# choderalab/pymbar

Hardware: NVIDIA H100
Metric: MBAR self-consistent iteration throughput at K=256, N=1e7 samples per GPU (u_kn entries/s; iter/s and HBM GB/s alongside) (higher is better)
Workload: dtype f64

## Files before the change

pymbar_b200/csrc/api.cu:

```cuda
#include <dlfcn.h>
#include <nccl.h>

#include <algorithm>
#include <cmath>
#include <cstring>

#include "internal.cuh"

using namespace mbar;

namespace mbar {

struct NcclApi {
    void* handle = nullptr;
    ncclResult_t (*GetUniqueId)(ncclUniqueId*) = nullptr;
    ncclResult_t (*CommInitRank)(ncclComm_t*, int, ncclUniqueId, int) = nullptr;
    ncclResult_t (*CommDestroy)(ncclComm_t) = nullptr;
    ncclResult_t (*AllReduce)(const void*, void*, size_t, ncclDataType_t, ncclRedOp_t, ncclComm_t,
                              cudaStream_t) = nullptr;
    const char* (*GetErrorString)(ncclResult_t) = nullptr;
};
static NcclApi g_nccl;

static int nccl_load() {
// ... 94 lines not shown
    const bool wantL = want.L || want.G || want.Gall;
    bool fused = false, wroteW = false;
    for (int attempt = 0; attempt < 3; ++attempt) {
        fused = false;
        wroteW = false;
        const bool logAll = (attempt == 2);
        if (attempt == 0 && c->kernelChoice != MBAR_B200_KERNEL_GENERIC)
            MBAR_TRY(launch_pass_fused(c, f, wantL, needUnsampled, &fused, want.G && !want.Gall, &wroteW));
        if (attempt == 0 && !fused) continue;
        if (!fused) MBAR_TRY(launch_pass_generic(c, f, wantL, logAll));
        MBAR_TRY(comm_allreduce(c, c->d_out, K + 2, 0));
        if (((needUnsampled && !fused) || logAll) && c->comm && c->nranks > 1) {
            double* mx = c->d_scratch;
            double* sc = c->d_scratch + K;
            MBAR_CUDA(cudaMemcpyAsync(mx, c->d_out + lay.logS(), K * sizeof(double),
                                      cudaMemcpyDeviceToDevice, c->stream));
            MBAR_TRY(comm_allreduce(c, mx, K, 2));
            logs_to_scaled<<<(K + 255) / 256, 256, 0, c->stream>>>(c->d_out + lay.logS(), mx, sc, K);
            MBAR_TRY(comm_allreduce(c, sc, K, 0));
            scaled_to_logs<<<(K + 255) / 256, 256, 0, c->stream>>>(c->d_out + lay.logS(), mx, sc, K);
            c->launches += 2;
        }
        MBAR_CUDA(cudaMemcpyAsync(c->h_out, c->d_out, (size_t)lay.size(false) * sizeof(double),
                                  cudaMemcpyDeviceToHost, c->stream));
        MBAR_CUDA(cudaStreamSynchronize(c->stream));
        c->d2hBytes += (int64_t)lay.size(false) * 8;
        float ms = 0.f;
        if (event_ms(c->evA, c->evB, &ms)) c->lastPassMs = ms;
        if (fused && c->h_out[lay.flag()] != 0.0) continue;
        if (fused && needUnsampled) {
            bool ok = true;
            for (int k = 0; k < K; ++k)
                if (!(c->h_Nk[k] > 0)) {
                    const double S = c->h_out[lay.S() + k];
                    if (!(S > 1e-250 && S < 1e12)) ok = false;
                    c->h_out[lay.logS() + k] = std::log(S);
                    c->h_out[lay.S() + k] = 0.0;
                }
            if (!ok) continue;
        }
        if (logAll) {
            for (int k : c->active) c->h_out[lay.S() + k] = std::exp(c->h_out[lay.logS() + k]);
            break;
        }
        bool underflow = false;
        for (int k : c->active) {
            const double S = c->h_out[lay.S() + k];
            if (!(S > 1e-280)) underflow = true;
            c->h_out[lay.logS() + k] = std::log(S);
        }
        if (!underflow) break;
        if (attempt == 0) ++attempt;
    }
    if (needUnsampled)
        for (int k = 0; k < K; ++k)
            if (!(c->h_Nk[k] > 0) && c->h_ufar[k] != 0.0 && c->h_uclamp[k] == 0.0) c->h_out[lay.logS() + k] = -INFINITY;
    if (want.G || want.Gall) {
        NvtxRange nvtxH("mbar_b200::hessian");
        MBAR_TRY(launch_hessian(c, f, want.Gall, fused && wroteW));
        MBAR_TRY(comm_allreduce(c, c->d_out + lay.G(), K * K, 0));
        MBAR_CUDA(cudaMemcpyAsync(c->h_out + lay.G(), c->d_out + lay.G(), (size_t)K * K * sizeof(double),
                                  cudaMemcpyDeviceToHost, c->stream));
        MBAR_CUDA(cudaStreamSynchronize(c->stream));
        c->d2hBytes += (int64_t)K * K * 8;
    }
    return MBAR_B200_OK;
}

double global_sumx(mbar_b200_ctx* c, int* rc) {
    *rc = MBAR_B200_OK;
    const double mine = c->d_wgt ? c->sumXw : c->sumX;
    if (!c->comm || c->nranks == 1) return mine;
    double* d = c->d_scratch;
    cudaMemcpyAsync(d, &mine, sizeof(double), cudaMemcpyHostToDevice, c->stream);
    *rc = comm_allreduce(c, d, 1, 0);
    double v = 0.0;
    cudaMemcpyAsync(&v, d, sizeof(double), cudaMemcpyDeviceToHost, c->stream);
    cudaStreamSynchronize(c->stream);
    return v;
}

}

extern "C" {

int mbar_b200_pass(mbar_b200_ctx* c, const double* f, double* S, double* sumL, double* G) {
    PassWant w;
    w.G = (G != nullptr);
    MBAR_TRY(run_pass(c, f, w));
    const int K = c->K;
    const PassLayout lay{K};
    if (S) std::memcpy(S, c->h_out + lay.S(), K * sizeof(double));
    if (sumL) {
        int rc;
        const double sx = global_sumx(c, &rc);
        MBAR_TRY(rc);
        *sumL = c->h_out[lay.sumL()] - sx;
    }
    if (G) {
        const double* Gh = c->h_out + lay.G();
        for (int i = 0; i < K; ++i)
            for (int j = 0; j < K; ++j) {
                const double d = c->h_Nk[i] * c->h_Nk[j];
                G[(size_t)i * K + j] = d > 0 ? Gh[(size_t)i * K + j] / d : 0.0;
            }
    }
    return MBAR_B200_OK;
}

int mbar_b200_pass_multi(mbar_b200_ctx* c, int32_t M, const double* f, double* S, double* sumL) {
    MBAR_REQUIRE(c && f, MBAR_B200_ERR_INVALID, "NULL argument");
    MBAR_REQUIRE(M >= 1 && M <= 2, MBAR_B200_ERR_INVALID, "M=%d: 1 or 2 candidates", M);
    MBAR_REQUIRE(c->ready, MBAR_B200_ERR_NOT_READY, "u_kn has not been uploaded");
    MBAR_REQUIRE(c->nranks == 1 || c->comm, MBAR_B200_ERR_NOT_READY, "sharded problem without a communicator");
    MBAR_CUDA(cudaSetDevice(c->device));
    const int K = c->K;
    const PassLayout lay{K};
    NvtxRange nvtx_("mbar_b200::pass_multi");
    for (int m = 0; m < M; ++m) MBAR_TRY(check_range(c, f + (size_t)m * K));
    int rc0;
    const double sx = global_sumx(c, &rc0);
    MBAR_TRY(rc0);
    bool fast = c->kernelChoice != MBAR_B200_KERNEL_GENERIC;
    FusedParams p[2];
    bool batched = false;
    static const bool noM2 = std::getenv("MBAR_B200_NO_M2") != nullptr;
    if (fast && M == 2 && !noM2) {
        bool ok0 = false, ok1 = false;
        MBAR_TRY(fused_prepare(c, f, false, false, &p[0], &ok0, c->dc(ROW_C), c->hf(ROW_C), false, 2));
        if (ok0)
            MBAR_TRY(fused_prepare(c, f + K, false, false, &p[1], &ok1, c->dc(ROW_C2), c->hf(ROW_C2), false, 2));
        if (ok0 && ok1) {
            p[0].c2 = p[1].c;
            p[0].mid2 = p[1].mid;
            p[0].out = c->d_outM;
            p[0].out2 = c->d_outM + lay.size(false);
            batched = true;
        }
    }
    for (int m = 0; m < M && fast && !batched; ++m) {
        bool ok = false;
        const int row = m == 0 ? ROW_C : ROW_C2;
        MBAR_TRY(fused_prepare(c, f + (size_t)m * K, false, false, &p[m], &ok, c->dc(row), c->hf(row)));
        p[m].out = c->d_outM + (size_t)m * lay.size(false);
        fast = ok;
    }
    if (fast) {
        if (batched) {
            MBAR_TRY(fused_enqueue(c, p[0]));
            MBAR_TRY(comm_allreduce(c, p[0].out, K + 2, 0));
            MBAR_TRY(comm_allreduce(c, p[0].out2, K + 2, 0));
        } else {
            for (int m = 0; m < M; ++m) {
                MBAR_TRY(fused_enqueue(c, p[m]));
                MBAR_TRY(comm_allreduce(c, p[m].out, K + 2, 0));
            }
        }
        MBAR_CUDA(cudaMemcpyAsync(c->h_out, c->d_outM, (size_t)M * lay.size(false) * sizeof(double),
                                  cudaMemcpyDeviceToHost, c->stream));
        MBAR_CUDA(cudaStreamSynchronize(c->stream));
        c->d2hBytes += (int64_t)M * lay.size(false) * 8;
        for (int m = 0; m < M && fast; ++m) {
            const double* o = c->h_out + (size_t)m * lay.size(false);
            if (o[lay.flag()] != 0.0) fast = false;
            for (int k : c->active)
                if (!(o[k] > 1e-280)) fast = false;
        }
        if (fast) {
            for (int m = 0; m < M; ++m) {
                const double* o = c->h_out + (size_t)m * lay.size(false);
                if (S)
                    for (int k = 0; k < K; ++k) S[(size_t)m * K + k] = c->h_Nk[k] > 0 ? o[k] : 0.0;
                if (sumL) sumL[m] = o[lay.sumL()] - sx;
            }
            return MBAR_B200_OK;
        }
    }
    for (int m = 0; m < M; ++m) {
        MBAR_TRY(run_pass(c, f + (size_t)m * K, PassWant{}));
        if (S) std::memcpy(S + (size_t)m * K, c->h_out + lay.S(), K * sizeof(double));
        if (sumL) sumL[m] = c->h_out[lay.sumL()] - sx;
    }
    return MBAR_B200_OK;
}

int mbar_b200_last_kernels(const mbar_b200_ctx* c, char* pass_kernel, char* hessian_kernel, int32_t len) {
    MBAR_REQUIRE(c && len > 0, MBAR_B200_ERR_INVALID, "bad argument");
    if (pass_kernel) snprintf(pass_kernel, (size_t)len, "%s", c->lastKernel);
    if (hessian_kernel) snprintf(hessian_kernel, (size_t)len, "%s", c->lastHessKernel);
    return MBAR_B200_OK;
}

int mbar_b200_last_hessian_ms(mbar_b200_ctx* c, double* weights_ms, double* hessian_ms) {
    MBAR_REQUIRE(c, MBAR_B200_ERR_INVALID, "ctx is NULL");
    MBAR_CUDA(cudaSetDevice(c->device));
    MBAR_CUDA(cudaStreamSynchronize(c->stream));
    float a = 0.f, b = 0.f;
    if (cudaEventElapsedTime(&a, c->evH0, c->evH1) != cudaSuccess) { cudaGetLastError(); a = 0.f; }
    if (cudaEventElapsedTime(&b, c->evH1, c->evH2) != cudaSuccess) { cudaGetLastError(); b = 0.f; }
    if (weights_ms) *weights_ms = a;
    if (hessian_ms) *hessian_ms = b;
    return MBAR_B200_OK;
}

int mbar_b200_self_consistent_update(mbar_b200_ctx* c, const double* f, double* f_out) {
    MBAR_REQUIRE(f_out, MBAR_B200_ERR_INVALID, "f_out is NULL");
    PassWant w;
    w.unsampled = true;
    MBAR_TRY(run_pass(c, f, w));
    const PassLayout lay{c->K};
    for (int k = 0; k < c->K; ++k) {
        f_out[k] = f[k] - c->h_out[lay.logS() + k];
    }
    return MBAR_B200_OK;
}

int mbar_b200_gradient(mbar_b200_ctx* c, const double* f, double* g_out) {
    MBAR_REQUIRE(g_out, MBAR_B200_ERR_INVALID, "g_out is NULL");
    MBAR_TRY(run_pass(c, f, PassWant{}));
    for (int k = 0; k < c->K; ++k) g_out[k] = c->h_Nk[k] * (c->h_out[k] - 1.0);
    return MBAR_B200_OK;
}

int mbar_b200_objective_and_gradient(mbar_b200_ctx* c, const double* f, double* obj, double* g_out) {
    MBAR_REQUIRE(obj, MBAR_B200_ERR_INVALID, "obj_out is NULL");
    MBAR_TRY(run_pass(c, f, PassWant{}));
    const PassLayout lay{c->K};
    int rc;
    const double sx = global_sumx(c, &rc);
    MBAR_TRY(rc);
    double nf = 0.0;
    for (int k = 0; k < c->K; ++k) nf += c->h_Nk[k] * f[k];
    *obj = (c->h_out[lay.sumL()] - sx) - nf;
    if (g_out)
        for (int k = 0; k < c->K; ++k) g_out[k] = c->h_Nk[k] * (c->h_out[k] - 1.0);
    return MBAR_B200_OK;
}

int mbar_b200_hessian(mbar_b200_ctx* c, const double* f, double* H) {
    MBAR_REQUIRE(H, MBAR_B200_ERR_INVALID, "H_out is NULL");
    PassWant w;
    w.G = true;
    MBAR_TRY(run_pass(c, f, w));
    const int K = c->K;
    const PassLayout lay{K};
    const double* Gh = c->h_out + lay.G();
    for (int i = 0; i < K; ++i)
        for (int j = 0; j < K; ++j) {
            double v = -Gh[(size_t)i * K + j];
            if (i == j) v += c->h_Nk[i] * c->h_out[lay.S() + i];
            H[(size_t)i * K + j] = (c->h_Nk[i] > 0 && c->h_Nk[j] > 0) ? v : 0.0;
        }
    return MBAR_B200_OK;
}

int mbar_b200_weight_moments(mbar_b200_ctx* c, const double* f, double* S, double* G) {
    MBAR_REQUIRE(G, MBAR_B200_ERR_INVALID, "G_out is NULL");
    PassWant w;
    w.unsampled = true;
    w.Gall = true;
    MBAR_TRY(run_pass(c, f, w));
    const int K = c->K;
    const PassLayout lay{K};
    const double* Gh = c->h_out + lay.G();
    for (int i = 0; i < K; ++i) {
        const double si = c->h_Nk[i] > 0 ? c->h_Nk[i] : 1.0;
        if (S) S[i] = c->h_Nk[i] > 0 ? c->h_out[lay.S() + i] : std::exp(c->h_out[lay.logS() + i]);
        for (int j = 0; j < K; ++j) {
            const double sj = c->h_Nk[j] > 0 ? c->h_Nk[j] : 1.0;
            G[(size_t)i * K + j] = Gh[(size_t)i * K + j] / (si * sj);
        }
    }
    return MBAR_B200_OK;
}

int mbar_b200_log_W_nk(mbar_b200_ctx* c, const double* f, double* logW, int64_t ld, int expo) {
    MBAR_REQUIRE(logW, MBAR_B200_ERR_INVALID, "logW_host is NULL");
    MBAR_REQUIRE(c && ld >= c->K, MBAR_B200_ERR_INVALID, "ld_out < K");
    PassWant w;
    w.L = true;
    MBAR_TRY(run_pass(c, f, w));
    return launch_logw(c, f, logW, ld, expo, 0, c->N);
}

int mbar_b200_log_W_nk_rows(mbar_b200_ctx* c, const double* f, int64_t n0, int64_t n, double* logW, int64_t ld,
                            int expo) {
    MBAR_REQUIRE(logW, MBAR_B200_ERR_INVALID, "logW_host is NULL");
    MBAR_REQUIRE(c && ld >= c->K, MBAR_B200_ERR_INVALID, "ld_out < K");
    MBAR_REQUIRE(n0 >= 0 && n >= 1 && n0 + n <= c->N && n0 % TILE_N == 0, MBAR_B200_ERR_INVALID,
                 "rows [%lld, +%lld): n0 must be a multiple of 32 inside [0, N_local)", (long long)n0, (long long)n);
    PassWant w;
    w.L = true;
    MBAR_TRY(run_pass(c, f, w));
    return launch_logw(c, f, logW, ld, expo, n0, n);
}

int mbar_b200_log_denominator(mbar_b200_ctx* c, const double* f, double* L_host) {
    MBAR_REQUIRE(L_host, MBAR_B200_ERR_INVALID, "L_host is NULL");
    PassWant w;
    w.L = true;
    MBAR_TRY(run_pass(c, f, w));
    std::vector<double> x((size_t)c->N);
    MBAR_CUDA(cudaMemcpyAsync(L_host, c->d_L, (size_t)c->N * sizeof(double), cudaMemcpyDeviceToHost, c->stream));
    MBAR_CUDA(cudaMemcpyAsync(x.data(), c->d_xshift, (size_t)c->N * sizeof(double), cudaMemcpyDeviceToHost, c->stream));
    MBAR_CUDA(cudaStreamSynchronize(c->stream));
    c->d2hBytes += 2 * c->N * 8;
// ... 99 lines not shown
```

pymbar_b200/csrc/ctx.cu:

```cuda
#include <cmath>
#include <cstring>
#include <algorithm>
#include <cstdlib>
#include <condition_variable>
#include <functional>
#include <mutex>
#include <thread>

#include <sys/syscall.h>
#include <unistd.h>

#include "internal.cuh"

namespace mbar {

static thread_local char g_err[512] = "";

namespace {
struct HostPool {
    std::vector<std::thread> workers;
    std::mutex m;
    std::condition_variable cvStart, cvDone;
    const std::function<void(int)>* fn = nullptr;
    int nTasks = 0, next = 0, running = 0;
    uint64_t generation = 0;
    bool stop = false;
    int width = 1;

    HostPool() {
        int hw = (int)std::thread::hardware_concurrency();
        width = std::max(1, std::min(16, hw));
        if (const char* v = std::getenv("MBAR_B200_HOST_THREADS")) width = std::max(1, std::min(64, std::atoi(v)));
        for (int t = 1; t < width; ++t) workers.emplace_back([this] { loop(); });
    }
    ~HostPool() {
        {
            std::lock_guard<std::mutex> g(m);
            stop = true;
        }
        cvStart.notify_all();
        for (auto& w : workers) w.join();
    }
    void drain(std::unique_lock<std::mutex>& lk) {
        while (next < nTasks) {
            const int i = next++;
            ++running;
            lk.unlock();
            (*fn)(i);
            lk.lock();
            --running;
        }
    }
    void loop() {
        std::unique_lock<std::mutex> lk(m);
        uint64_t seen = 0;
        for (;;) {
            cvStart.wait(lk, [&] { return stop || generation != seen; });
            if (stop) return;
            seen = generation;
            drain(lk);
            if (running == 0 && next >= nTasks) cvDone.notify_all();
        }
    }
    void run(int n, const std::function<void(int)>& f) {
        std::unique_lock<std::mutex> lk(m);
        fn = &f;
        nTasks = n;
        next = 0;
        ++generation;
        cvStart.notify_all();
        drain(lk);
        cvDone.wait(lk, [&] { return running == 0 && next >= nTasks; });
        fn = nullptr;
    }
};
HostPool& pool() {
    static HostPool p;
    return p;
}
std::mutex g_poolUse;
}

void host_parallel(int nTasks, const std::function<void(int)>& fn) {
    if (nTasks <= 1) {
        for (int i = 0; i < nTasks; ++i) fn(i);
        return;
    }
    std::lock_guard<std::mutex> g(g_poolUse);
    pool().run(nTasks, fn);
}
int host_parallel_width() { return pool().width; }

int gpu_numa_node(int device) {
    static int cache[16] = {-2, -2, -2, -2, -2, -2, -2, -2, -2, -2, -2, -2, -2, -2, -2, -2};
    int& c = cache[device & 15];
    if (c != -2) return c;
    c = -1;
    char bus[32] = "";
    if (cudaDeviceGetPCIBusId(bus, sizeof(bus), device) != cudaSuccess) {
        cudaGetLastError();
        return c;
    }
    for (char* q = bus; *q; ++q)
        if (*q >= 'A' && *q <= 'F') *q = (char)(*q - 'A' + 'a');
    char path[128];
    snprintf(path, sizeof(path), "/sys/bus/pci/devices/%s/numa_node", bus);
    if (FILE* fh = fopen(path, "r")) {
        int node = -1;
        if (fscanf(fh, "%d", &node) == 1) c = node;
        fclose(fh);
    }
    return c;
}
NumaPrefer::NumaPrefer(int device) {
#if defined(SYS_set_mempolicy)
    const int node = gpu_numa_node(device);
    if (node < 0 || node >= 1024) return;
    unsigned long mask[16] = {0};
    mask[node / (8 * sizeof(unsigned long))] |= 1ul << (node % (8 * sizeof(unsigned long)));
    if (syscall(SYS_set_mempolicy, 1, mask, (unsigned long)(sizeof(mask) * 8)) == 0) active = true;
#else
    (void)device;
#endif
}
NumaPrefer::~NumaPrefer() {
#if defined(SYS_set_mempolicy)
    if (active) syscall(SYS_set_mempolicy, 0 , nullptr, 0ul);
#endif
}

void set_error(const char* fmt, ...) {
    va_list ap;
    va_start(ap, fmt);
    vsnprintf(g_err, sizeof(g_err), fmt, ap);
    va_end(ap);
}

struct Parked {
    void* ptr = nullptr;
    size_t bytes = 0;
};
struct DevicePool {
    Parked u, stageDev[2], stagePin[2];
};
static DevicePool g_pool[16];
static std::mutex g_poolMutex;
static bool pool_enabled() {
    static const bool off = std::getenv("MBAR_B200_NO_POOL") != nullptr;
    return !off;
}
static void* pool_take(Parked& slot, size_t bytes) {
    std::lock_guard<std::mutex> g(g_poolMutex);
    if (slot.ptr && slot.bytes >= bytes && slot.bytes <= 2 * bytes + (1u << 20)) {
        void* p = slot.ptr;
        slot = Parked{};
        return p;
    }
    return nullptr;
}
static void* pool_park(Parked& slot, void* ptr, size_t bytes) {
    std::lock_guard<std::mutex> g(g_poolMutex);
    void* old = slot.ptr;
    slot.ptr = ptr;
    slot.bytes = bytes;
    return old;
}

__device__ __forceinline__ void row_min_push(int* rowMin, double v, int lane) {
    int vi = v < 0.0 ? (int)fmax(floor(v), -1073741824.0) : 0;
    vi = __reduce_min_sync(0xffffffffu, vi);
    if (lane == 0 && vi < 0) atomicMin(rowMin, vi);
}
__device__ __forceinline__ void row_clamp_push(int* rowClamp, unsigned long long* rowFar, double d, bool valid,
                                               int lane) {
    const unsigned far = __ballot_sync(0xffffffffu, valid && d >= U_NEAR_CLAMP);
    if (far == 0u) return;
    const bool finite = __any_sync(0xffffffffu, valid && d >= U_NEAR_CLAMP && d < INFINITY);
    if (lane == 0) {
        atomicAdd(rowFar, (unsigned long long)__popc(far));
        if (finite) atomicOr(rowClamp, 1);
    }
}

enum { BAD_NAN = 1, BAD_NO_FINITE = 2, BAD_NEG_INF = 4 };
static const char* upload_error(int flags) {
    return flags & BAD_NAN ? "u_kn contains NaN"
         : flags & BAD_NO_FINITE ? "a sample has no finite energy in any sampled state"
                                 : "an unsampled state has an energy of -inf (its free energy would be -inf)";
}

__global__ void __launch_bounds__(256) retile_kernel(const double* __restrict__ src, int64_t ld,
                                                     int K, int64_t tile0, int64_t validCols,
                                                     const unsigned long long* __restrict__ rowmask,
                                                     double* __restrict__ dst,
                                                     double* __restrict__ xshift,
                                                     int* __restrict__ flags, int* __restrict__ urowmin,
                                                     unsigned long long* __restrict__ urowfar) {
    __shared__ double s_min[8][TILE_N];
    __shared__ int s_bad[8];
    const int lane = threadIdx.x & 31, warp = threadIdx.x >> 5;
    const int64_t tileLocal = blockIdx.x;
    const int64_t col = tileLocal * TILE_N + lane;
    const bool valid = col < validCols;
    const double* colp = src + col;

    double mn = INFINITY;
    unsigned bad = 0;
    for (int k = warp; k < K; k += 8) {
        double v = valid ? colp[(int64_t)k * ld] : 0.0;
        if (v != v) bad |= BAD_NAN;
        const bool act = (rowmask[k >> 6] >> (k & 63)) & 1ull;
        if (act) mn = fmin(mn, v);
        else if (v == -INFINITY) bad |= BAD_NEG_INF;
    }
    s_min[warp][lane] = mn;
    bad = __reduce_or_sync(0xffffffffu, bad);
    if (lane == 0) s_bad[warp] = (int)bad;
    __syncthreads();
    double x = s_min[0][lane];
#pragma unroll
    for (int w = 1; w < 8; ++w) x = fmin(x, s_min[w][lane]);
    int anyBad = 0;
#pragma unroll
    for (int w = 0; w < 8; ++w) anyBad |= s_bad[w];
    const bool finiteShift = isfinite(x);
    if (valid && !finiteShift && warp == 0) atomicOr(&flags[0], BAD_NO_FINITE);
    if (!valid || !finiteShift) x = 0.0;

    double* out = dst + (tile0 + tileLocal) * (int64_t)K * TILE_N + lane;
    for (int k = warp; k < K; k += 8) {
        double v = valid ? colp[(int64_t)k * ld] : 0.0;
        const double d = v - x;
        row_clamp_push(urowmin + K + k, urowfar + k, d, valid, lane);
        v = fmin(d, U_CLAMP);
        row_min_push(urowmin + k, valid ? v : 0.0, lane);
        out[(int64_t)k * TILE_N] = valid ? v : 0.0;
    }
    if (warp == 0) xshift[(tile0 + tileLocal) * TILE_N + lane] = x;
    if (anyBad && threadIdx.x == 0) atomicOr(&flags[0], anyBad);
}

int retile_chunk(mbar_b200_ctx* ctx, const double* d_rowmajor, int64_t ldCols, int64_t tile0,
                 int64_t nTilesChunk, int64_t validCols, cudaStream_t s) {
    if (nTilesChunk <= 0) return MBAR_B200_OK;
    retile_kernel<<<(unsigned)nTilesChunk, 256, 0, s>>>(d_rowmajor, ldCols, ctx->K, tile0, validCols,
                                                       ctx->d_rowmask, ctx->d_u, ctx->d_xshift,
                                                       ctx->d_flag, ctx->d_urowmin, ctx->d_urowfar);
    ctx->launches++;
    MBAR_CUDA(cudaGetLastError());
    return MBAR_B200_OK;
}

__global__ void __launch_bounds__(256) untile_kernel(const double* __restrict__ u,
                                                     const double* __restrict__ xshift, int K,
                                                     int64_t n0, int64_t n, double* __restrict__ dst,
                                                     int64_t ld) {
    const int lane = threadIdx.x & 31, warp = threadIdx.x >> 5;
    const int64_t j = (int64_t)blockIdx.x * TILE_N + lane;
    if (j >= n) return;
    const int64_t g = n0 + j;
    const int64_t tile = g / TILE_N;
    const int l = (int)(g % TILE_N);
    const double x = xshift[g];
    for (int k = warp; k < K; k += 8)
        dst[(int64_t)k * ld + j] = u[(tile * K + k) * TILE_N + l] + x;
}

int launch_untile(mbar_b200_ctx* ctx, int64_t n0, int64_t n, double* d_dst, int64_t ld) {
    const unsigned grid = (unsigned)((n + TILE_N - 1) / TILE_N);
    untile_kernel<<<grid, 256, 0, ctx->stream>>>(ctx->d_u, ctx->d_xshift, ctx->K, n0, n, d_dst, ld);
    ctx->launches++;
    MBAR_CUDA(cudaGetLastError());
    return MBAR_B200_OK;
}

__global__ void __launch_bounds__(256) sumx_kernel(const double* __restrict__ x, int64_t N,
                                                   double* __restrict__ partial) {
    __shared__ double s[8];
    double acc = 0.0;
    for (int64_t i = (int64_t)blockIdx.x * blockDim.x + threadIdx.x; i < N;
         i += (int64_t)gridDim.x * blockDim.x)
        acc += x[i];
    acc = warp_sum(acc);
    if ((threadIdx.x & 31) == 0) s[threadIdx.x >> 5] = acc;
    __syncthreads();
    if (threadIdx.x == 0) {
        double t = 0.0;
        for (int w = 0; w < 8; ++w) t += s[w];
        partial[blockIdx.x] = t;
    }
}

__global__ void __launch_bounds__(256) wprep_kernel(const double* __restrict__ w, const double* __restrict__ x,
                                                    int64_t N, double* __restrict__ sqrtw,
                                                    double* __restrict__ partial) {
    __shared__ double s[8];
    double acc = 0.0;
    for (int64_t i = (int64_t)blockIdx.x * blockDim.x + threadIdx.x; i < N;
         i += (int64_t)gridDim.x * blockDim.x) {
        const double wi = w[i];
        sqrtw[i] = sqrt(wi);
        acc += wi * x[i];
    }
    acc = warp_sum(acc);
    if ((threadIdx.x & 31) == 0) s[threadIdx.x >> 5] = acc;
    __syncthreads();
    if (threadIdx.x == 0) {
        double t = 0.0;
        for (int i = 0; i < 8; ++i) t += s[i];
        partial[blockIdx.x] = t;
    }
}

int set_weights(mbar_b200_ctx* ctx, const double* w_host) {
    if (!w_host) {
        cudaFree(ctx->d_wgt);
        cudaFree(ctx->d_sqrtw);
        ctx->d_wgt = ctx->d_sqrtw = nullptr;
// ... 138 lines not shown
}

int open_device(int device, cudaDeviceProp* propOut) {
    int ndev = 0;
    if (cudaGetDeviceCount(&ndev) != cudaSuccess || ndev == 0) {
        cudaGetLastError();
        set_error("no CUDA device visible: libmbar_b200 has no CPU fallback");
        return MBAR_B200_ERR_NO_DEVICE;
    }
    MBAR_REQUIRE(device >= 0 && device < ndev, MBAR_B200_ERR_INVALID, "device %d of %d", device, ndev);
    MBAR_CUDA(cudaSetDevice(device));
    cudaDeviceProp prop;
    MBAR_CUDA(cudaGetDeviceProperties(&prop, device));
    if (prop.major != 9 || prop.minor != 0) {
        set_error("device %d is sm_%d%d; this library is built for sm_90a (H100) only", device,
                  prop.major, prop.minor);
        return MBAR_B200_ERR_NO_DEVICE;
    }
    if (propOut) *propOut = prop;
    return MBAR_B200_OK;
}

}

using namespace mbar;

extern "C" {

int mbar_b200_abi_version(void) { return MBAR_B200_ABI_VERSION; }
const char* mbar_b200_last_error(void) { return g_err; }

int mbar_b200_device_count(int* count) {
    MBAR_REQUIRE(count, MBAR_B200_ERR_INVALID, "count is NULL");
    int n = 0;
    cudaError_t e = cudaGetDeviceCount(&n);
    if (e != cudaSuccess) {
        cudaGetLastError();
        n = 0;
    }
    *count = n;
    return MBAR_B200_OK;
}

int mbar_b200_host_alloc(void** ptr, uint64_t bytes) {
    MBAR_REQUIRE(ptr, MBAR_B200_ERR_INVALID, "ptr is NULL");
    int dev = 0;
    cudaGetDevice(&dev);
    NumaPrefer numa(dev);
    MBAR_CUDA(cudaHostAlloc(ptr, bytes, cudaHostAllocDefault));
    return MBAR_B200_OK;
}
int mbar_b200_host_free(void* ptr) {
    if (ptr) MBAR_CUDA(cudaFreeHost(ptr));
    return MBAR_B200_OK;
}

static inline uint64_t mix64(uint64_t h, uint64_t w) {
    h ^= w;
    h *= 0x9E3779B97F4A7C15ull;
    return h ^ (h >> 29);
}
static uint64_t hash_span(const unsigned char* p, size_t bytes, uint64_t seed) {
    uint64_t h0 = seed, h1 = seed ^ 0xD6E8FEB86659FD93ull, h2 = seed + 0xA0761D6478BD642Full, h3 = ~seed;
    size_t i = 0;
    for (; i + 32 <= bytes; i += 32) {
        uint64_t w[4];
        std::memcpy(w, p + i, 32);
        h0 = mix64(h0, w[0]);
        h1 = mix64(h1, w[1]);
        h2 = mix64(h2, w[2]);
        h3 = mix64(h3, w[3]);
    }
    for (; i < bytes; ++i) h0 = mix64(h0, p[i]);
    return mix64(mix64(mix64(h0, h1), h2), h3);
}

int mbar_b200_host_hash(const void* base, int64_t rows, int64_t row_bytes, int64_t stride_bytes, uint64_t* out) {
    MBAR_REQUIRE(base && out && rows >= 0 && row_bytes >= 0 && stride_bytes >= row_bytes, MBAR_B200_ERR_INVALID,
                 "bad argument");
    const unsigned char* b = static_cast<const unsigned char*>(base);
    const int64_t blk = 4ll << 20;
    const int64_t perRow = row_bytes ? (row_bytes + blk - 1) / blk : 0;
    const int64_t nBlocks = rows * perRow;
    std::vector<uint64_t> part((size_t)nBlocks);
    host_parallel((int)std::min<int64_t>(nBlocks, 1 << 30), [&](int i) {
        const int64_t r = i / perRow, c = i % perRow;
        const int64_t off = c * blk, len = std::min(blk, row_bytes - off);
        part[(size_t)i] = hash_span(b + r * stride_bytes + off, (size_t)len, 0x243F6A8885A308D3ull + (uint64_t)i);
    });
    uint64_t h = 0x13198A2E03707344ull ^ (uint64_t)rows ^ ((uint64_t)row_bytes << 20);
    for (uint64_t v : part) h = mix64(h, v);
    *out = h;
    return MBAR_B200_OK;
}

int mbar_b200_create(mbar_b200_ctx** out, int device, int32_t K, int64_t N_local, const double* N_k) {
    MBAR_REQUIRE(out && N_k, MBAR_B200_ERR_INVALID, "NULL argument");
    *out = nullptr;
    MBAR_REQUIRE(K >= 1 && K <= MBAR_B200_MAX_STATES, MBAR_B200_ERR_INVALID, "K=%d outside [1, %d]", K,
                 MBAR_B200_MAX_STATES);
    MBAR_REQUIRE(N_local >= 1, MBAR_B200_ERR_INVALID, "N_local=%lld must be >= 1", (long long)N_local);
    cudaDeviceProp prop;
    MBAR_TRY(open_device(device, &prop));
    mbar_b200_ctx* c = new mbar_b200_ctx();
    c->device = device;
    c->K = K;
    c->N = N_local;
    c->nTiles = (N_local + TILE_N - 1) / TILE_N;
    c->smCount = prop.multiProcessorCount;
    c->h_Nk.assign(N_k, N_k + K);
    c->h_logNk.resize(K);
    c->h_logNkEff.resize(K);
    std::vector<unsigned long long> mask((K + 63) / 64, 0ull);
    for (int k = 0; k < K; ++k) {
        if (!(N_k[k] >= 0.0)) {
            delete c;
            set_error("N_k[%d]=%g is negative or NaN", k, N_k[k]);
            return MBAR_B200_ERR_INVALID;
        }
        c->N_total_states += N_k[k];
        if (N_k[k] > 0) {
            c->active.push_back(k);
            mask[k >> 6] |= 1ull << (k & 63);
            c->h_logNk[k] = std::log(N_k[k]);
            c->h_logNkEff[k] = c->h_logNk[k];
        } else {
            c->h_logNk[k] = -INFINITY;
            c->h_logNkEff[k] = LOG_EPS_UNSAMPLED;
        }
    }
    if (c->active.empty()) {
        delete c;
        set_error("all N_k are zero");
        return MBAR_B200_ERR_INVALID;
    }
    c->firstActive = c->active[0];

    const size_t uBytes = (size_t)c->nTiles * K * TILE_N * sizeof(double);
    const size_t nPad = (size_t)c->nTiles * TILE_N;
    const PassLayout lay{K};
#define ALLOC(p, bytes)                                                        \
    do {                                                                       \
        cudaError_t e = cudaMalloc((void**)&(p), (bytes));                     \
        if (e != cudaSuccess) {                                                \
            set_error("cudaMalloc(%zu bytes) failed: %s", (size_t)(bytes), cudaGetErrorString(e)); \
            mbar_b200_destroy(c);                                              \
            return MBAR_B200_ERR_NOMEM;                                        \
        }                                                                      \
    } while (0)
    c->uBytes = uBytes;
    if (pool_enabled()) {
        c->d_u = static_cast<double*>(pool_take(g_pool[device & 15].u, uBytes));
        if (c->d_u) c->uBytes = 0;
    }
    if (!c->d_u) ALLOC(c->d_u, uBytes);
    ALLOC(c->d_xshift, nPad * sizeof(double));
    ALLOC(c->d_c, DC_ROWS * (size_t)K * sizeof(double));
    ALLOC(c->d_Nk, (size_t)K * sizeof(double));
    ALLOC(c->d_NkEff, (size_t)K * sizeof(double));
    ALLOC(c->d_rowmask, mask.size() * sizeof(unsigned long long));
    ALLOC(c->d_zeromask, mask.size() * sizeof(unsigned long long));
    ALLOC(c->d_onesmask, mask.size() * sizeof(unsigned long long));
    ALLOC(c->d_partial, (size_t)MAX_GRID * (3 * (size_t)K + 2) * sizeof(double));
    ALLOC(c->d_out, (size_t)lay.size(true) * sizeof(double));
    ALLOC(c->d_ticket, 4 * sizeof(unsigned int));
    ALLOC(c->d_flag, 4 * sizeof(int));
    ALLOC(c->d_urowmin, 2 * (size_t)K * sizeof(int));
    ALLOC(c->d_urowfar, (size_t)K * sizeof(unsigned long long));
    c->h_urowmin.assign(K, 0.0);
    c->h_uclamp.assign(K, 0.0);
    c->h_ufar.assign(K, 0.0);
    ALLOC(c->d_f, (size_t)K * sizeof(double));
    ALLOC(c->d_scratch, (scratch_rendezvous(K) + 1024) * sizeof(double));
    ALLOC(c->d_loop, sizeof(mbar::LoopState));
    ALLOC(c->d_av, 8 * (size_t)K * sizeof(double));
    ALLOC(c->d_outM, 2 * (size_t)lay.size(false) * sizeof(double));
    ALLOC(c->d_A, (size_t)K * K * sizeof(double));
    ALLOC(c->d_active, (size_t)K * sizeof(int));
    ALLOC(c->d_seq, sizeof(unsigned long long));
#undef ALLOC
#define CREATE_CUDA(call)                                                                   \
    do {                                                                                    \
        cudaError_t e__ = (call);                                                           \
        if (e__ != cudaSuccess) {                                                           \
            set_error("%s failed at %s:%d: %s", #call, __FILE__, __LINE__,                  \
                      cudaGetErrorString(e__));                                             \
            mbar_b200_destroy(c);                                                           \
            return MBAR_B200_ERR_CUDA;                                                      \
        }                                                                                   \
    } while (0)
    CREATE_CUDA(cudaHostAlloc((void**)&c->h_loop, sizeof(mbar::LoopState), cudaHostAllocDefault));
    CREATE_CUDA(cudaMemset(c->d_loop, 0, sizeof(mbar::LoopState)));
    CREATE_CUDA(cudaMemset(c->d_seq, 0, sizeof(unsigned long long)));
    CREATE_CUDA(cudaMemcpy(c->d_active, c->active.data(), c->active.size() * sizeof(int), cudaMemcpyHostToDevice));
    CREATE_CUDA(cudaEventCreate(&c->evH0));
    CREATE_CUDA(cudaEventCreate(&c->evH1));
    CREATE_CUDA(cudaEventCreate(&c->evH2));
    CREATE_CUDA(cudaHostAlloc((void**)&c->h_out,
                              (size_t)std::max(lay.size(true), 2 * lay.size(false)) * sizeof(double),
                              cudaHostAllocDefault));
    CREATE_CUDA(cudaHostAlloc((void**)&c->h_f, HF_ROWS * (size_t)K * sizeof(double), cudaHostAllocDefault));
    CREATE_CUDA(cudaStreamCreateWithFlags(&c->stream, cudaStreamNonBlocking));
    CREATE_CUDA(cudaStreamCreateWithFlags(&c->copyStream, cudaStreamNonBlocking));
    CREATE_CUDA(cudaEventCreate(&c->evA));
    CREATE_CUDA(cudaEventCreate(&c->evB));
    CREATE_CUDA(cudaEventCreateWithFlags(&c->evCopy[0], cudaEventDisableTiming));
    CREATE_CUDA(cudaEventCreateWithFlags(&c->evCopy[1], cudaEventDisableTiming));
    CREATE_CUDA(cudaMemcpy(c->d_Nk, N_k, (size_t)K * sizeof(double), cudaMemcpyHostToDevice));
    {
        std::vector<double> eff(K);
        for (int k = 0; k < K; ++k) eff[k] = std::exp(c->h_logNkEff[k]);
        CREATE_CUDA(cudaMemcpy(c->d_NkEff, eff.data(), (size_t)K * sizeof(double), cudaMemcpyHostToDevice));
    }
    CREATE_CUDA(cudaMemcpy(c->d_rowmask, mask.data(), mask.size() * sizeof(unsigned long long),
                         cudaMemcpyHostToDevice));
    CREATE_CUDA(cudaMemset(c->d_zeromask, 0, mask.size() * sizeof(unsigned long long)));
    CREATE_CUDA(cudaMemset(c->d_onesmask, 0xff, mask.size() * sizeof(unsigned long long)));
    CREATE_CUDA(cudaMemset(c->d_ticket, 0, 4 * sizeof(unsigned int)));
    CREATE_CUDA(cudaMemset(c->d_flag, 0, 4 * sizeof(int)));
    CREATE_CUDA(cudaMemset(c->d_urowmin, 0, 2 * (size_t)K * sizeof(int)));
    CREATE_CUDA(cudaMemset(c->d_urowfar, 0, (size_t)K * sizeof(unsigned long long)));
#undef CREATE_CUDA
    *out = c;
    return MBAR_B200_OK;
}

int mbar_b200_destroy(mbar_b200_ctx* c) {
    if (!c) return MBAR_B200_OK;
    cudaSetDevice(c->device);
    if (c->comm) mbar_b200_comm_destroy(c);
    for (void* pm : c->peerMapped) cudaIpcCloseMemHandle(pm);
    cudaFree(c->d_inbox);
    if (c->stream) cudaStreamSynchronize(c->stream);
    if (pool_enabled() && c->d_u) {
        const size_t need = (size_t)c->nTiles * c->K * TILE_N * sizeof(double);
        cudaFree(pool_park(g_pool[c->device & 15].u, c->d_u, c->uBytes ? c->uBytes : need));
        for (int i = 0; i < 2; ++i) {
            const size_t sb = (size_t)c->stageCols * c->K * sizeof(double);
            if (c->stage_dev[i]) cudaFree(pool_park(g_pool[c->device & 15].stageDev[i], c->stage_dev[i], sb));
            if (c->stage_pinned[i]) {
                void* old = pool_park(g_pool[c->device & 15].stagePin[i], c->stage_pinned[i], sb);
                if (old) cudaFreeHost(old);
            }
            c->stage_dev[i] = nullptr;
            c->stage_pinned[i] = nullptr;
        }
    } else {
        cudaFree(c->d_u);
    }
    cudaFree(c->d_xshift); cudaFree(c->d_wgt); cudaFree(c->d_sqrtw); cudaFree(c->d_c); cudaFree(c->d_Nk); cudaFree(c->d_NkEff);
    cudaFree(c->d_rowmask); cudaFree(c->d_zeromask); cudaFree(c->d_onesmask); cudaFree(c->d_partial); cudaFree(c->d_out); cudaFree(c->d_L);
    cudaFree(c->d_W); cudaFree(c->d_ticket); cudaFree(c->d_flag); cudaFree(c->d_urowmin); cudaFree(c->d_urowfar); cudaFree(c->d_f);
    cudaFree(c->d_scratch);
    cudaFree(c->d_loop); cudaFree(c->d_av); cudaFree(c->d_outM); cudaFree(c->d_A); cudaFree(c->d_active);
    cudaFree(c->d_seq); cudaFree(c->d_Wt);
    if (c->loopGraph) cudaGraphExecDestroy(c->loopGraph);
    if (c->h_loop) cudaFreeHost(c->h_loop);
    if (c->evH0) cudaEventDestroy(c->evH0);
    if (c->evH1) cudaEventDestroy(c->evH1);
    if (c->evH2) cudaEventDestroy(c->evH2);
    for (int i = 0; i < 2; ++i) {
        if (c->stage_pinned[i]) cudaFreeHost(c->stage_pinned[i]);
        cudaFree(c->stage_dev[i]);
        if (c->evCopy[i]) cudaEventDestroy(c->evCopy[i]);
    }
    if (c->h_out) cudaFreeHost(c->h_out);
    if (c->h_f) cudaFreeHost(c->h_f);
    if (c->evA) cudaEventDestroy(c->evA);
    if (c->evB) cudaEventDestroy(c->evB);
    if (c->stream) cudaStreamDestroy(c->stream);
    if (c->copyStream) cudaStreamDestroy(c->copyStream);
    cudaGetLastError();
    delete c;
    return MBAR_B200_OK;
}

int mbar_b200_trim(void) {
    int cur = 0;
    cudaGetDevice(&cur);
    for (int d = 0; d < 16; ++d) {
        DevicePool old;
        {
            std::lock_guard<std::mutex> g(g_poolMutex);
            old = g_pool[d];
            g_pool[d] = DevicePool{};
        }
        if (!old.u.ptr && !old.stageDev[0].ptr && !old.stageDev[1].ptr && !old.stagePin[0].ptr &&
            !old.stagePin[1].ptr)
            continue;
        cudaSetDevice(d);
        cudaFree(old.u.ptr);
        for (int i = 0; i < 2; ++i) {
            cudaFree(old.stageDev[i].ptr);
            if (old.stagePin[i].ptr) cudaFreeHost(old.stagePin[i].ptr);
        }
    }
    cudaSetDevice(cur);
    cudaGetLastError();
    return MBAR_B200_OK;
}

int mbar_b200_get_shape(const mbar_b200_ctx* c, int32_t* K, int64_t* N_local) {
    MBAR_REQUIRE(c, MBAR_B200_ERR_INVALID, "ctx is NULL");
    if (K) *K = c->K;
    if (N_local) *N_local = c->N;
    return MBAR_B200_OK;
}

int mbar_b200_set_pass_kernel(mbar_b200_ctx* c, int kernel) {
    MBAR_REQUIRE(c, MBAR_B200_ERR_INVALID, "ctx is NULL");
    MBAR_REQUIRE(kernel >= 0 && kernel <= 2, MBAR_B200_ERR_INVALID, "kernel=%d", kernel);
    c->kernelChoice = kernel;
    return MBAR_B200_OK;
}

int mbar_b200_get_counters(const mbar_b200_ctx* c, int64_t* launches, int64_t* passes,
                           int64_t* h2d, int64_t* d2h) {
    MBAR_REQUIRE(c, MBAR_B200_ERR_INVALID, "ctx is NULL");
    if (launches) *launches = c->launches;
    if (passes) *passes = c->passes;
    if (h2d) *h2d = c->h2dBytes;
    if (d2h) *d2h = c->d2hBytes;
    return MBAR_B200_OK;
}

int mbar_b200_last_pass_ms(mbar_b200_ctx* c, double* ms) {
    MBAR_REQUIRE(c && ms, MBAR_B200_ERR_INVALID, "NULL argument");
    cudaSetDevice(c->device);
    float t = 0.f;
    if (c->stream && cudaStreamSynchronize(c->stream) == cudaSuccess && event_ms(c->evA, c->evB, &t))
        c->lastPassMs = t;
    else
        cudaGetLastError();
    *ms = c->lastPassMs;
    return MBAR_B200_OK;
}

static int ensure_staging(mbar_b200_ctx* c, bool needPinned) {
    if (c->stageCols == 0) {
        int64_t cols = (64ll << 20) / (8ll * c->K);
        cols = (cols / TILE_N) * TILE_N;
        if (cols < TILE_N) cols = TILE_N;
        const int64_t padN = c->nTiles * TILE_N;
        if (cols > padN) cols = padN;
        c->stageCols = cols;
    }
    const size_t bytes = (size_t)c->stageCols * c->K * sizeof(double);
    for (int i = 0; i < 2; ++i) {
        if (!c->stage_dev[i] && pool_enabled())
            c->stage_dev[i] = static_cast<double*>(pool_take(g_pool[c->device & 15].stageDev[i], bytes));
        if (!c->stage_dev[i]) MBAR_CUDA(cudaMalloc((void**)&c->stage_dev[i], bytes));
        if (needPinned && !c->stage_pinned[i] && pool_enabled())
            c->stage_pinned[i] = static_cast<double*>(pool_take(g_pool[c->device & 15].stagePin[i], bytes));
        if (needPinned && !c->stage_pinned[i]) {
            NumaPrefer numa(c->device);
            MBAR_CUDA(cudaHostAlloc((void**)&c->stage_pinned[i], bytes, cudaHostAllocDefault));
        }
    }
    return MBAR_B200_OK;
}

static int reset_row_stats(mbar_b200_ctx* c) {
    MBAR_CUDA(cudaMemset(c->d_urowmin, 0, 2 * (size_t)c->K * sizeof(int)));
    MBAR_CUDA(cudaMemset(c->d_urowfar, 0, (size_t)c->K * sizeof(unsigned long long)));
    return MBAR_B200_OK;
}

static int collect_row_minima(mbar_b200_ctx* c) {
    std::vector<int> m(2 * (size_t)c->K);
    std::vector<unsigned long long> far(c->K);
    MBAR_CUDA(cudaMemcpy(m.data(), c->d_urowmin, m.size() * sizeof(int), cudaMemcpyDeviceToHost));
    MBAR_CUDA(cudaMemcpy(far.data(), c->d_urowfar, far.size() * sizeof(unsigned long long), cudaMemcpyDeviceToHost));
    MBAR_TRY(reset_row_stats(c));
    for (int k = 0; k < c->K; ++k) {
        c->h_urowmin[k] = (double)m[k];
        c->h_uclamp[k] = (double)m[c->K + k];
        c->h_ufar[k] = far[k] == (unsigned long long)c->N ? 1.0 : 0.0;
    }
    return agree_row_minima(c);
}

static int finish_upload(mbar_b200_ctx* c) {
    int flags[4];
    MBAR_CUDA(cudaStreamSynchronize(c->copyStream));
    MBAR_CUDA(cudaStreamSynchronize(c->stream));
    MBAR_CUDA(cudaMemcpy(flags, c->d_flag, sizeof(flags), cudaMemcpyDeviceToHost));
    if (flags[0]) {
        MBAR_CUDA(cudaMemset(c->d_flag, 0, 4 * sizeof(int)));
        MBAR_TRY(reset_row_stats(c));
        c->ready = false;
        set_error("%s", upload_error(flags[0]));
        return MBAR_B200_ERR_NAN;
    }
    MBAR_TRY(reduce_sumx(c));
    MBAR_TRY(reduce_sumxw(c));
    MBAR_TRY(collect_row_minima(c));
    c->ready = true;
    return MBAR_B200_OK;
}

int mbar_b200_gpu_numa_node(int device, int* node) {
    MBAR_REQUIRE(node, MBAR_B200_ERR_INVALID, "node is NULL");
    *node = gpu_numa_node(device);
    return MBAR_B200_OK;
}

int mbar_b200_upload_u_kn(mbar_b200_ctx* c, const double* u_host, int64_t ld) {
    MBAR_REQUIRE(c && u_host, MBAR_B200_ERR_INVALID, "NULL argument");
    NvtxRange nvtx_("mbar_b200::upload_u_kn");
    MBAR_REQUIRE(ld >= c->N, MBAR_B200_ERR_INVALID, "ld=%lld < N_local=%lld", (long long)ld,
                 (long long)c->N);
    MBAR_CUDA(cudaSetDevice(c->device));
    cudaPointerAttributes attr;
    bool pinned = false;
    if (cudaPointerGetAttributes(&attr, u_host) == cudaSuccess)
        pinned = (attr.type == cudaMemoryTypeHost);
    else
        cudaGetLastError();
    MBAR_TRY(ensure_staging(c, !pinned));
    const int K = c->K;
    const int64_t cols = c->stageCols;
    int buf = 0;
    for (int64_t n0 = 0; n0 < c->N; n0 += cols, buf ^= 1) {
        const int64_t w = (c->N - n0 < cols) ? (c->N - n0) : cols;
        MBAR_CUDA(cudaStreamWaitEvent(c->copyStream, c->evCopy[buf], 0));
        const double* src = u_host + n0;
        int64_t srcLd = ld;
        if (!pinned) {
            MBAR_CUDA(cudaEventSynchronize(c->evCopy[buf]));
            double* p = c->stage_pinned[buf];
            if ((size_t)w * K < (1u << 16)) {
                for (int k = 0; k < K; ++k)
                    std::memcpy(p + (size_t)k * w, u_host + (size_t)k * ld + n0, (size_t)w * sizeof(double));
            } else {
                const int64_t piece = 16384;
                const int64_t perRow = (w + piece - 1) / piece;
                host_parallel((int)(K * perRow), [&](int task) {
                    const int64_t k = task / perRow, c0 = (task % perRow) * piece;
                    const int64_t len = std::min(piece, w - c0);
                    std::memcpy(p + (size_t)k * w + c0, u_host + (size_t)k * ld + n0 + c0, (size_t)len * sizeof(double));
                });
            }
            src = p;
            srcLd = w;
        }
        MBAR_CUDA(cudaMemcpy2DAsync(c->stage_dev[buf], (size_t)cols * sizeof(double), src,
                                    (size_t)srcLd * sizeof(double), (size_t)w * sizeof(double), K,
                                    cudaMemcpyHostToDevice, c->copyStream));
        c->h2dBytes += (int64_t)w * K * 8;
        cudaEvent_t copied;
        MBAR_CUDA(cudaEventCreateWithFlags(&copied, cudaEventDisableTiming));
        MBAR_CUDA(cudaEventRecord(copied, c->copyStream));
        MBAR_CUDA(cudaStreamWaitEvent(c->stream, copied, 0));
        MBAR_CUDA(cudaEventDestroy(copied));
        const int64_t nT = (w + TILE_N - 1) / TILE_N;
        MBAR_TRY(retile_chunk(c, c->stage_dev[buf], cols, n0 / TILE_N, nT, w, c->stream));
        MBAR_CUDA(cudaEventRecord(c->evCopy[buf], c->stream));
    }
    return finish_upload(c);
}

__global__ void __launch_bounds__(256) widen_tiles_kernel(const double* __restrict__ src, int K, int Knew,
                                                          int64_t nTiles, double* __restrict__ dst) {
    const int lane = threadIdx.x & 31, warp = threadIdx.x >> 5;
    for (int64_t tile = blockIdx.x; tile < nTiles; tile += gridDim.x) {
        const double* s = src + tile * (int64_t)K * TILE_N + lane;
        double* d = dst + tile * (int64_t)Knew * TILE_N + lane;
#pragma unroll 4
        for (int k = warp; k < K; k += 8) d[(int64_t)k * TILE_N] = s[(int64_t)k * TILE_N];
    }
}
__global__ void __launch_bounds__(256) append_rows_kernel(const double* __restrict__ stage, int64_t ldCols, int E,
                                                          int K, int Knew, int64_t tile0, int64_t validCols,
                                                          const double* __restrict__ xshift,
                                                          double* __restrict__ dst, int* __restrict__ flags,
                                                          int* __restrict__ urowmin,
                                                          unsigned long long* __restrict__ urowfar) {
    const int lane = threadIdx.x & 31, warp = threadIdx.x >> 5;
    const int64_t tl = blockIdx.x;
    const int64_t col = tl * TILE_N + lane;
    const bool valid = col < validCols;
    const double x = xshift[(tile0 + tl) * TILE_N + lane];
    double* out = dst + (tile0 + tl) * (int64_t)Knew * TILE_N + (int64_t)K * TILE_N + lane;
    unsigned bad = 0;
    for (int r = warp; r < E; r += 8) {
        double v = valid ? stage[(int64_t)r * ldCols + col] : 0.0;
        if (v != v) bad |= BAD_NAN;
        if (v == -INFINITY) bad |= BAD_NEG_INF;
        const double d = v - x;
        row_clamp_push(urowmin + Knew + K + r, urowfar + K + r, d, valid, lane);
        v = fmin(d, U_CLAMP);
        row_min_push(urowmin + K + r, valid ? v : 0.0, lane);
        out[(int64_t)r * TILE_N] = valid ? v : 0.0;
    }
    bad = __reduce_or_sync(0xffffffffu, bad);
    if (bad && lane == 0) atomicOr(&flags[0], (int)bad);
}

int mbar_b200_create_augmented(mbar_b200_ctx* base, int32_t n_extra, const double* u_extra_host, int64_t ld,
                               mbar_b200_ctx** out) {
    MBAR_REQUIRE(base && u_extra_host && out, MBAR_B200_ERR_INVALID, "NULL argument");
    *out = nullptr;
    MBAR_REQUIRE(base->ready, MBAR_B200_ERR_NOT_READY, "base problem has no u_kn yet");
    MBAR_REQUIRE(n_extra >= 1 && base->K + n_extra <= MBAR_B200_MAX_STATES, MBAR_B200_ERR_INVALID,
                 "n_extra=%d: K + n_extra must lie in [K + 1, %d]", n_extra, MBAR_B200_MAX_STATES);
    MBAR_REQUIRE(ld >= base->N, MBAR_B200_ERR_INVALID, "ld=%lld < N_local", (long long)ld);
    NvtxRange nvtx_("mbar_b200::create_augmented");
    const int K = base->K, E = n_extra, Kn = K + E;
    std::vector<double> Nk(base->h_Nk);
    Nk.resize(Kn, 0.0);
    mbar_b200_ctx* c = nullptr;
    MBAR_TRY(mbar_b200_create(&c, base->device, Kn, base->N, Nk.data()));
    auto fail = [&](int rc) {
        mbar_b200_destroy(c);
        return rc;
    };
#define AUG_CUDA(call)                                                                         \
    do {                                                                                       \
        cudaError_t e__ = (call);                                                              \
        if (e__ != cudaSuccess) {                                                              \
            set_error("%s failed at %s:%d: %s", #call, __FILE__, __LINE__, cudaGetErrorString(e__)); \
            return fail(MBAR_B200_ERR_CUDA);                                                   \
        }                                                                                      \
    } while (0)
    AUG_CUDA(cudaStreamSynchronize(base->stream));
    const size_t nPad = (size_t)c->nTiles * TILE_N;
    AUG_CUDA(cudaMemcpyAsync(c->d_xshift, base->d_xshift, nPad * sizeof(double), cudaMemcpyDeviceToDevice, c->stream));
    c->sumX = base->sumX;
    {
        int64_t grid = (int64_t)c->smCount * 8;
        if (grid > c->nTiles) grid = c->nTiles;
        widen_tiles_kernel<<<(unsigned)grid, 256, 0, c->stream>>>(base->d_u, K, Kn, c->nTiles, c->d_u);
        c->launches++;
        AUG_CUDA(cudaGetLastError());
    }
    int64_t cols = (32ll << 20) / (8ll * E);
    cols = (cols / TILE_N) * TILE_N;
    if (cols < TILE_N) cols = TILE_N;
    if (cols > (int64_t)nPad) cols = (int64_t)nPad;
    cudaPointerAttributes attr;
    bool pinned = false;
    if (cudaPointerGetAttributes(&attr, u_extra_host) == cudaSuccess)
        pinned = (attr.type == cudaMemoryTypeHost);
    else
        cudaGetLastError();
    double* d_stage = nullptr;
    double* h_stage = nullptr;
    AUG_CUDA(cudaMalloc((void**)&d_stage, (size_t)cols * E * sizeof(double)));
    if (!pinned) {
        NumaPrefer numa(c->device);
        cudaError_t e = cudaHostAlloc((void**)&h_stage, (size_t)cols * E * sizeof(double), cudaHostAllocDefault);
        if (e != cudaSuccess) {
            cudaFree(d_stage);
            set_error("cudaHostAlloc failed: %s", cudaGetErrorString(e));
            return fail(MBAR_B200_ERR_NOMEM);
        }
    }
    int rc = MBAR_B200_OK;
    for (int64_t n0 = 0; n0 < c->N && rc == MBAR_B200_OK; n0 += cols) {
        const int64_t w = (c->N - n0 < cols) ? (c->N - n0) : cols;
        const double* src = u_extra_host + n0;
        int64_t srcLd = ld;
        if (!pinned) {
            cudaStreamSynchronize(c->stream);
            for (int r = 0; r < E; ++r)
                std::memcpy(h_stage + (size_t)r * w, u_extra_host + (size_t)r * ld + n0, (size_t)w * sizeof(double));
            src = h_stage;
            srcLd = w;
        }
        cudaError_t e = cudaMemcpy2DAsync(d_stage, (size_t)cols * sizeof(double), src, (size_t)srcLd * sizeof(double),
                                          (size_t)w * sizeof(double), E, cudaMemcpyHostToDevice, c->stream);
        if (e != cudaSuccess) {
            set_error("append rows: H2D failed: %s", cudaGetErrorString(e));
            rc = MBAR_B200_ERR_CUDA;
            break;
        }
        c->h2dBytes += (int64_t)w * E * 8;
        const int64_t nT = (w + TILE_N - 1) / TILE_N;
        append_rows_kernel<<<(unsigned)nT, 256, 0, c->stream>>>(d_stage, cols, E, K, Kn, n0 / TILE_N, w,
                                                              c->d_xshift, c->d_u, c->d_flag, c->d_urowmin,
                                                              c->d_urowfar);
        c->launches++;
        if (pinned) cudaStreamSynchronize(c->stream);
    }
    cudaStreamSynchronize(c->stream);
    cudaFree(d_stage);
    if (h_stage) cudaFreeHost(h_stage);
    if (rc != MBAR_B200_OK) return fail(rc);
    int flags[4] = {0, 0, 0, 0};
    AUG_CUDA(cudaMemcpy(flags, c->d_flag, sizeof(flags), cudaMemcpyDeviceToHost));
    AUG_CUDA(cudaMemset(c->d_flag, 0, 4 * sizeof(int)));
    if (flags[0]) {
        set_error(flags[0] & BAD_NAN ? "appended energies contain NaN"
                                     : "an appended state has an energy of -inf (its free energy would be -inf)");
        return fail(MBAR_B200_ERR_NAN);
    }
    {
        std::vector<int> m(2 * (size_t)Kn);
        std::vector<unsigned long long> far(Kn);
        AUG_CUDA(cudaMemcpy(m.data(), c->d_urowmin, m.size() * sizeof(int), cudaMemcpyDeviceToHost));
        AUG_CUDA(cudaMemcpy(far.data(), c->d_urowfar, far.size() * sizeof(unsigned long long), cudaMemcpyDeviceToHost));
        if (reset_row_stats(c) != MBAR_B200_OK) return fail(MBAR_B200_ERR_CUDA);
        for (int k = 0; k < K; ++k) {
            c->h_urowmin[k] = base->h_urowmin[k];
            c->h_uclamp[k] = base->h_uclamp[k];
            c->h_ufar[k] = base->h_ufar[k];
        }
        for (int r = 0; r < E; ++r) {
            c->h_urowmin[K + r] = (double)m[K + r];
            c->h_uclamp[K + r] = (double)m[Kn + K + r];
            c->h_ufar[K + r] = far[K + r] == (unsigned long long)c->N ? 1.0 : 0.0;
        }
    }
    if (base->d_wgt) {
        AUG_CUDA(cudaMalloc((void**)&c->d_wgt, nPad * sizeof(double)));
        AUG_CUDA(cudaMalloc((void**)&c->d_sqrtw, nPad * sizeof(double)));
        AUG_CUDA(cudaMemcpy(c->d_wgt, base->d_wgt, nPad * sizeof(double), cudaMemcpyDeviceToDevice));
        AUG_CUDA(cudaMemcpy(c->d_sqrtw, base->d_sqrtw, nPad * sizeof(double), cudaMemcpyDeviceToDevice));
        c->sumW = base->sumW;
        c->sumXw = base->sumXw;
    }
#undef AUG_CUDA
    c->ready = true;
    *out = c;
    return MBAR_B200_OK;
}

int mbar_b200_upload_u_kn_dev(mbar_b200_ctx* c, const double* u_dev, int64_t ld) {
    MBAR_REQUIRE(c && u_dev, MBAR_B200_ERR_INVALID, "NULL argument");
    MBAR_REQUIRE(ld >= c->N, MBAR_B200_ERR_INVALID, "ld=%lld < N_local", (long long)ld);
    MBAR_CUDA(cudaSetDevice(c->device));
    MBAR_CUDA(cudaDeviceSynchronize());
    MBAR_TRY(retile_chunk(c, u_dev, ld, 0, c->nTiles, c->N, c->stream));
    return finish_upload(c);
}

int mbar_b200_synthesize(mbar_b200_ctx* c, const mbar_b200_synth* spec) {
    MBAR_REQUIRE(c && spec && spec->O_k && spec->k_k, MBAR_B200_ERR_INVALID, "NULL argument");
    MBAR_CUDA(cudaSetDevice(c->device));
    MBAR_TRY(launch_synth(c, spec));
    MBAR_TRY(reduce_sumx(c));
    MBAR_TRY(reduce_sumxw(c));
    MBAR_TRY(collect_row_minima(c));
    c->ready = true;
    return MBAR_B200_OK;
}

int mbar_b200_set_sample_weights(mbar_b200_ctx* c, const double* w_host) {
    MBAR_REQUIRE(c, MBAR_B200_ERR_INVALID, "ctx is NULL");
    MBAR_REQUIRE(c->ready, MBAR_B200_ERR_NOT_READY, "u_kn not uploaded");
    MBAR_CUDA(cudaSetDevice(c->device));
    return set_weights(c, w_host);
}

int mbar_b200_download_u_kn(mbar_b200_ctx* c, int64_t n0, int64_t n, double* u_host, int64_t ld) {
    MBAR_REQUIRE(c && u_host, MBAR_B200_ERR_INVALID, "NULL argument");
    MBAR_REQUIRE(c->ready, MBAR_B200_ERR_NOT_READY, "u_kn not uploaded");
    MBAR_REQUIRE(n0 >= 0 && n >= 1 && n0 + n <= c->N && ld >= n, MBAR_B200_ERR_INVALID,
                 "bad slice [%lld, +%lld) ld=%lld", (long long)n0, (long long)n, (long long)ld);
    MBAR_CUDA(cudaSetDevice(c->device));
    const int64_t maxCols = (32ll << 20) / (8ll * c->K) / TILE_N * TILE_N + TILE_N;
    double* d_tmp = nullptr;
    const int64_t cols = n < maxCols ? n : maxCols;
    MBAR_CUDA(cudaMalloc((void**)&d_tmp, (size_t)cols * c->K * sizeof(double)));
    int rc = MBAR_B200_OK;
    for (int64_t j = 0; j < n && rc == MBAR_B200_OK; j += cols) {
        const int64_t w = (n - j < cols) ? (n - j) : cols;
        rc = launch_untile(c, n0 + j, w, d_tmp, cols);
        if (rc != MBAR_B200_OK) break;
        cudaError_t e = cudaMemcpy2DAsync(u_host + j, (size_t)ld * sizeof(double), d_tmp,
                                          (size_t)cols * sizeof(double), (size_t)w * sizeof(double),
                                          c->K, cudaMemcpyDeviceToHost, c->stream);
        if (e == cudaSuccess) e = cudaStreamSynchronize(c->stream);
        if (e != cudaSuccess) {
            set_error("download failed: %s", cudaGetErrorString(e));
            rc = MBAR_B200_ERR_CUDA;
        }
        c->d2hBytes += (int64_t)w * c->K * 8;
    }
    cudaFree(d_tmp);
    return rc;
}

}
```

pymbar_b200/csrc/hessian.cu:

```cuda
#include <cmath>
#include <cstdlib>
#include <vector>

#include "internal.cuh"

namespace mbar {

constexpr int HB = 128;
constexpr int HNS = 3;
constexpr uint32_t HPANEL = HB * TILE_N * 8;

__device__ __forceinline__ void dmma884(double& c0, double& c1, double a, double b) {
    asm volatile("mma.sync.aligned.m8n8k4.row.col.f64.f64.f64.f64 {%0,%1}, {%2}, {%3}, {%0,%1};"
                 : "+d"(c0), "+d"(c1)
                 : "d"(a), "d"(b));
}

__device__ __forceinline__ void convert_row(double* P, int row, int lane, double ck, bool act, bool valid,
                                            double L, const double* tab, double sw) {
    const double v = P[row * TILE_N + lane];
    __syncwarp();
    double wv = 0.0;
    if (valid && act) wv = sw * exp_fast(fmin(fmax(ck - v - L, -800.0), 700.0), tab);
    P[row * TILE_N + (lane ^ ((row & 7) << 2))] = wv;
// ... 358 lines not shown
    constexpr int KP = KT * 8;
    constexpr int NT = KT * (KT + 1) / 2;
    extern __shared__ __align__(128) unsigned char smem_raw[];
    double* tab = reinterpret_cast<double*>(smem_raw);
    uint64_t* bar_full = reinterpret_cast<uint64_t*>(tab + 32);
    uint64_t* bar_empty = bar_full + 32;
    unsigned char* ring = smem_raw + 1024;
    const uint32_t slotBytes = KP * TILE_N * 8;
    const int lane = threadIdx.x & 31, warp = threadIdx.x >> 5;
    const int q = warp >> 1, h = warp & 1;

    const int64_t t0 = nTiles * blockIdx.x / gridDim.x, t1 = nTiles * (blockIdx.x + 1) / gridDim.x;
    const int n = (int)(t1 - t0);
    if (threadIdx.x < 32) tab[threadIdx.x] = MBAR_EXP_TABLE[threadIdx.x];
    if (threadIdx.x == 0) {
        for (int i = 0; i < NSLOT; ++i) {
            mbar_init(smem_u32(&bar_full[i]), 1);
            mbar_init(smem_u32(&bar_empty[i]), 2);
        }
        mbar_fence_init();
    }
    __syncthreads();

    const uint32_t tileBytes = (uint32_t)K * TILE_N * 8;
    auto issue = [&](int j) {
        const int slot = j % NSLOT;
        const uint32_t fb = smem_u32(&bar_full[slot]);
        mbar_arrive_expect_tx(fb, tileBytes);
        bulk_g2s(smem_u32(ring + (size_t)slot * slotBytes), u + (t0 + j) * (int64_t)K * TILE_N, tileBytes, fb);
    };
    if (h == 0 && lane == 0)
        for (int j = q; j < n && j < NSLOT; j += 4) issue(j);

    const int fragCol = lane & 3, fragRow = lane >> 2;
    double cr[KT];
    uint32_t act = 0;
#pragma unroll
    for (int mt = 0; mt < KT; ++mt) {
        const int k = mt * 8 + fragRow;
        const bool a = k < K && (WIN || ((rowmask[k >> 6] >> (k & 63)) & 1ull));
        cr[mt] = (a && !WIN) ? c[k] : 0.0;
        act |= (uint32_t)a << mt;
    }
    double acc[NT][2];
#pragma unroll
    for (int i = 0; i < NT; ++i) acc[i][0] = acc[i][1] = 0.0;

    for (int j = q; j < n; j += 4) {
        const int slot = j % NSLOT;
        const uint32_t par = (uint32_t)(j / NSLOT) & 1u;
        const int64_t tile = t0 + j;
        double Lt = 0.0, swt = 1.0;
        if (!WIN) {
            Lt = Lp[tile * TILE_N + lane];
            if (sqrtw) swt = sqrtw[tile * TILE_N + lane];
        }
        mbar_wait(smem_u32(&bar_full[slot]), par);
        const double* P = reinterpret_cast<const double*>(ring + (size_t)slot * slotBytes);
#pragma unroll
        for (int kk = 0; kk < 4; ++kk) {
            const int ks = 4 * h + kk;
            const int s = ks * 4 + fragCol;
            double a[KT];
            if (WIN) {
                const int col = ((ks ^ fragRow) << 2) + fragCol;
#pragma unroll
                for (int mt = 0; mt < KT; ++mt) {
                    const double v = P[(mt * 8 + fragRow) * TILE_N + col];
                    a[mt] = ((act >> mt) & 1u) ? v : 0.0;
                }
            } else {
                const double L = __shfl_sync(0xffffffffu, Lt, s);
                const double sw = __shfl_sync(0xffffffffu, swt, s);
                const bool valid = tile * TILE_N + s < N;
#pragma unroll
                for (int mt = 0; mt < KT; ++mt) {
                    const double v = P[(mt * 8 + fragRow) * TILE_N + s];
                    const double e = sw * exp_fast(fmin(fmax(cr[mt] - v - L, -800.0), 700.0), tab);
                    a[mt] = (valid && ((act >> mt) & 1u)) ? e : 0.0;
                }
            }
#pragma unroll
            for (int mt = 0; mt < KT; ++mt)
#pragma unroll
                for (int nt = 0; nt <= mt; ++nt)
                    dmma884(acc[mt * (mt + 1) / 2 + nt][0], acc[mt * (mt + 1) / 2 + nt][1], a[mt], a[nt]);
        }
        __syncwarp();
        if (lane == 0) mbar_arrive(smem_u32(&bar_empty[slot]));
        if (h == 0 && lane == 0 && j + NSLOT < n) {
            mbar_wait(smem_u32(&bar_empty[slot]), par);
            issue(j + NSLOT);
        }
    }
    __syncthreads();
    double* red = reinterpret_cast<double*>(ring);
    for (int w2 = 0; w2 < 8; ++w2) {
        if (warp == w2) {
#pragma unroll
            for (int mt = 0; mt < KT; ++mt)
#pragma unroll
                for (int nt = 0; nt <= mt; ++nt) {
                    const int row = mt * 8 + (lane >> 2), col = nt * 8 + (lane & 3) * 2;
                    const int idx = mt * (mt + 1) / 2 + nt;
                    if (w2 == 0) {
                        red[row * KP + col] = acc[idx][0];
                        red[row * KP + col + 1] = acc[idx][1];
                    } else {
                        red[row * KP + col] += acc[idx][0];
                        red[row * KP + col + 1] += acc[idx][1];
                    }
                }
        }
        __syncthreads();
    }
    double* out = Gpart + (size_t)blockIdx.x * KP * KP;
    for (int e = threadIdx.x; e < KP * KP; e += blockDim.x)
        if (((e / KP) >> 3) >= ((e % KP) >> 3)) out[e] = red[e];
}

__global__ void __launch_bounds__(256)
hessian_small_reduce_kernel(const double* __restrict__ Gpart, int K, int KP, int nCtas, double* __restrict__ G,
                            const LoopState* loop) {
    if (loop && *reinterpret_cast<const volatile int*>(&loop->done)) return;
    for (int e = blockIdx.x * blockDim.x + threadIdx.x; e < KP * KP; e += gridDim.x * blockDim.x) {
        const int i = e / KP, j = e % KP;
        if (i >= K || j >= K || (i >> 3) < (j >> 3)) continue;
        double s = 0.0;
        for (int b = 0; b < nCtas; ++b) s += Gpart[(size_t)b * KP * KP + e];
        G[(size_t)i * K + j] = s;
        if ((i >> 3) > (j >> 3)) G[(size_t)j * K + i] = s;
    }
}

static int ensure_gpart(mbar_b200_ctx* ctx, size_t bytes) {
    static_assert(sizeof(size_t) == 8, "64-bit build");
    if (ctx->d_W && ctx->gpartBytes >= bytes) return MBAR_B200_OK;
    if (ctx->d_W) cudaFree(ctx->d_W);
    ctx->d_W = nullptr;
    MBAR_CUDA(cudaMalloc((void**)&ctx->d_W, bytes));
    ctx->gpartBytes = bytes;
    return MBAR_B200_OK;
}

bool ensure_weight_buffer(mbar_b200_ctx* ctx) {
    static const bool forceOld = std::getenv("MBAR_B200_HESSIAN_INPLACE") != nullptr;
    if (forceOld) return false;
    if (ctx->d_Wt) return true;
    if (ctx->wtAllocFailed) return false;
    const size_t bytes = (size_t)ctx->nTiles * ctx->K * TILE_N * sizeof(double);
    if (cudaMalloc((void**)&ctx->d_Wt, bytes) != cudaSuccess) {
        cudaGetLastError();
        ctx->d_Wt = nullptr;
        ctx->wtAllocFailed = true;
        return false;
    }
    return true;
}

int launch_hessian_dev(mbar_b200_ctx* ctx, const double* d_ch, bool allRows, LoopState* loop, bool weightsReady) {
    const int K = ctx->K;
    MBAR_REQUIRE(ctx->d_L, MBAR_B200_ERR_NOT_READY, "hessian: per-sample L not available");
    const PassLayout lay{K};
    const unsigned long long* mask = allRows ? ctx->d_onesmask : ctx->d_rowmask;
    static const bool forceOld = std::getenv("MBAR_B200_HESSIAN_INPLACE") != nullptr;
    if (!ctx->capturing) MBAR_CUDA(cudaEventRecord(ctx->evH0, ctx->stream));
    if (K <= 64 && !forceOld) {
        const int KT = K <= 16 ? 2 : K <= 32 ? 4 : 8;
        const int KP = KT * 8;
        const size_t slotBytes = (size_t)KP * TILE_N * 8;
        int nslot = (int)((200 * 1024) / slotBytes) & ~3;
        if (nslot > 32) nslot = 32;
        int64_t grid = ctx->smCount;
        if (grid > (ctx->nTiles + 3) / 4) grid = (ctx->nTiles + 3) / 4;
        if (grid < 1) grid = 1;
        MBAR_TRY(ensure_gpart(ctx, (size_t)grid * KP * KP * sizeof(double)));
        const size_t smem = 1024 + (size_t)nslot * slotBytes;
        const bool win = weightsReady && !allRows && ctx->d_Wt;
        void (*kern)(const double*, const double*, const double*, const unsigned long long*, int, int64_t, int64_t,
                     int, double*, const double*, const LoopState*) =
            win ? (KT == 2 ? hessian_small_kernel<2, true> : KT == 4 ? hessian_small_kernel<4, true>
                                                                     : hessian_small_kernel<8, true>)
                : (KT == 2 ? hessian_small_kernel<2, false> : KT == 4 ? hessian_small_kernel<4, false>
                                                                      : hessian_small_kernel<8, false>);
        static size_t attr[16][6] = {{0}};
        size_t& a = attr[ctx->device & 15][(KT == 2 ? 0 : KT == 4 ? 1 : 2) + (win ? 3 : 0)];
        if (a < smem) {
            MBAR_CUDA(cudaFuncSetAttribute(kern, cudaFuncAttributeMaxDynamicSharedMemorySize, (int)smem));
            a = smem;
        }
        if (!ctx->capturing) MBAR_CUDA(cudaEventRecord(ctx->evH1, ctx->stream));
        kern<<<(unsigned)grid, 256, smem, ctx->stream>>>(win ? ctx->d_Wt : ctx->d_u, ctx->d_L, d_ch, mask, K, ctx->N,
                                                        ctx->nTiles, nslot, ctx->d_W, ctx->d_sqrtw, loop);
        MBAR_CUDA(cudaGetLastError());
        hessian_small_reduce_kernel<<<(KP * KP + 255) / 256, 256, 0, ctx->stream>>>(ctx->d_W, K, KP, (int)grid,
                                                                                    ctx->d_out + lay.G(), loop);
        MBAR_CUDA(cudaGetLastError());
        if (!ctx->capturing) MBAR_CUDA(cudaEventRecord(ctx->evH2, ctx->stream));
        snprintf(ctx->lastHessKernel, sizeof(ctx->lastHessKernel), "hessian_small_kernel<KT=%d, %s> grid=%lld NSLOT=%d",
                 KT, win ? "weights stored by the fused pass (WST)" : "in-register conversion", (long long)grid, nslot);
        ctx->launches += 2;
        ctx->passes++;
        return MBAR_B200_OK;
    }

    const int nB = (K + HB - 1) / HB;
    const int nPairsAll = nB * (nB + 1) / 2;
    const bool materialise = !forceOld && ensure_weight_buffer(ctx);
    const double wOff = materialise ? 64.0 : 4.0, wDiag = materialise ? 36.0 : 3.0;
    static bool attr[16][2] = {{false}};
    const size_t smem = 512 + (size_t)HNS * 2 * HPANEL;
    if (materialise && !(weightsReady && !allRows)) {
        int64_t wgrid = (int64_t)ctx->smCount * 8;
        if (wgrid > ctx->nTiles) wgrid = ctx->nTiles;
        weights_kernel<<<(unsigned)wgrid, 256, 0, ctx->stream>>>(ctx->d_u, ctx->d_L, d_ch, mask, K, ctx->N,
                                                                ctx->nTiles, ctx->d_sqrtw, ctx->d_Wt, loop);
        MBAR_CUDA(cudaGetLastError());
        ctx->launches++;
    }
    if (!ctx->capturing) MBAR_CUDA(cudaEventRecord(ctx->evH1, ctx->stream));
    int totalCtas = 0;
    for (int base = 0; base < nPairsAll; base += 128) {
        const int nPairs = std::min(128, nPairsAll - base);
        HessSplit split{};
        split.nPairs = nPairs;
        split.pairBase = base;
        std::vector<char> isDiag(nPairs);
        {
            int bi = 0, rem = base;
            while (rem > bi) { rem -= bi + 1; ++bi; }
            int bj = rem;
            for (int p = 0; p < nPairs; ++p) {
                isDiag[p] = (bi == bj);
                if (++bj > bi) { ++bi; bj = 0; }
            }
        }
        double wsum = 0.0;
        for (int p = 0; p < nPairs; ++p) wsum += isDiag[p] ? wDiag : wOff;
        const int total = ctx->smCount > nPairs ? ctx->smCount : nPairs;
        int used = 0;
        std::vector<int> cnt(nPairs);
        std::vector<double> frac(nPairs);
        for (int p = 0; p < nPairs; ++p) {
            const double x = total * (isDiag[p] ? wDiag : wOff) / wsum;
            cnt[p] = (int)x;
            if (cnt[p] < 1) cnt[p] = 1;
            frac[p] = x - (int)x;
            used += cnt[p];
        }
        while (used < total) {
            int best = 0;
            for (int p = 1; p < nPairs; ++p)
                if (frac[p] > frac[best]) best = p;
            cnt[best]++;
            frac[best] = -1.0;
            used++;
        }
        used = 0;
        for (int p = 0; p < nPairs; ++p) {
            if ((int64_t)cnt[p] > ctx->nTiles) cnt[p] = (int)ctx->nTiles;
            split.pairStart[p] = used;
            used += cnt[p];
        }
        split.pairStart[nPairs] = used;
        const int nCtas = used;
        totalCtas += nCtas;
        MBAR_TRY(ensure_gpart(ctx, (size_t)nCtas * HB * HB * sizeof(double)));
        if (materialise) {
            if (!attr[ctx->device & 15][0]) {
                MBAR_CUDA(cudaFuncSetAttribute(hessian_big_kernel, cudaFuncAttributeMaxDynamicSharedMemorySize, (int)smem));
                attr[ctx->device & 15][0] = true;
            }
            hessian_big_kernel<<<nCtas, 512, smem, ctx->stream>>>(ctx->d_Wt, K, ctx->nTiles, split, ctx->d_W, loop);
            MBAR_CUDA(cudaGetLastError());
            hessian_big_reduce_kernel<<<dim3(nPairs, 16), 256, 0, ctx->stream>>>(ctx->d_W, K, split,
                                                                                ctx->d_out + lay.G(), loop);
            MBAR_CUDA(cudaGetLastError());
        } else {
            if (!attr[ctx->device & 15][1]) {
                MBAR_CUDA(cudaFuncSetAttribute(hessian_inplace_kernel, cudaFuncAttributeMaxDynamicSharedMemorySize, (int)smem));
                attr[ctx->device & 15][1] = true;
            }
            hessian_inplace_kernel<<<nCtas, 512, smem, ctx->stream>>>(ctx->d_u, ctx->d_L, d_ch, mask, K, ctx->N,
                                                                     ctx->nTiles, split, ctx->d_W, ctx->d_sqrtw, loop);
            MBAR_CUDA(cudaGetLastError());
            hessian_reduce_kernel<<<dim3(nPairs, 16), 256, 0, ctx->stream>>>(ctx->d_W, K, split, ctx->d_out + lay.G(),
                                                                            loop);
            MBAR_CUDA(cudaGetLastError());
        }
        ctx->launches += 2;
    }
    if (materialise)
        snprintf(ctx->lastHessKernel, sizeof(ctx->lastHessKernel),
                 "%s + hessian_big_kernel (128x128 block pairs: %d, CTAs %d)",
                 (weightsReady && !allRows) ? "weights stored by the fused pass (WST)" : "weights_kernel", nPairsAll,
                 totalCtas);
    else
        snprintf(ctx->lastHessKernel, sizeof(ctx->lastHessKernel), "hessian_inplace_kernel (round 1), CTAs %d", totalCtas);
    if (!ctx->capturing) MBAR_CUDA(cudaEventRecord(ctx->evH2, ctx->stream));
    ctx->passes++;
    return MBAR_B200_OK;
}

int launch_hessian(mbar_b200_ctx* ctx, const double* h_f, bool allRows, bool weightsReady) {
    const int K = ctx->K;
    double* c = ctx->hf(ROW_HESS_C);
// ... 9 lines not shown
```

pymbar_b200/csrc/internal.cuh:

```cuda
#pragma once
#include <cuda_runtime.h>
#include <stdint.h>

#include <cstdarg>
#include <cstdio>
#include <functional>
#include <vector>

#include "../../include/mbar_b200.h"
#include "exp_tables.h"

namespace mbar {

constexpr int TILE_N = 32;
constexpr double U_CLAMP = 1.0e6;
constexpr double U_NEAR_CLAMP = U_CLAMP - 800.0;
constexpr double C_RANGE = 1.0e6;
constexpr double FUSED_SPREAD = 1200.0;
constexpr int MAX_GRID = 132 * 4;
constexpr double LOG_EPS_UNSAMPLED = -80.0;
constexpr double FUSED_MAX_ARG = 700.0;
constexpr double LOG_FLOOR_S = -670.273323601467;

void set_error(const char* fmt, ...);
#define MBAR_CUDA(call)                                                                     \
    do {                                                                                    \
        cudaError_t e__ = (call);                                                           \
        if (e__ != cudaSuccess) {                                                           \
            mbar::set_error("%s failed at %s:%d: %s", #call, __FILE__, __LINE__,            \
                            cudaGetErrorString(e__));                                       \
            return MBAR_B200_ERR_CUDA;                                                      \
        }                                                                                   \
    } while (0)
#define MBAR_REQUIRE(cond, status, ...)                                                     \
    do {                                                                                    \
        if (!(cond)) {                                                                      \
            mbar::set_error(__VA_ARGS__);                                                   \
            return (status);                                                                \
        }                                                                                   \
    } while (0)
#define MBAR_TRY(call)                                                                      \
    do {                                                                                    \
        int s__ = (call);                                                                   \
        if (s__ != MBAR_B200_OK) return s__;                                                \
    } while (0)

struct PassLayout {
    int K;
    __host__ __device__ int S() const { return 0; }
    __host__ __device__ int sumL() const { return K; }
    __host__ __device__ int flag() const { return K + 1; }
    __host__ __device__ int logS() const { return K + 2; }
    __host__ __device__ int G() const { return 2 * K + 2; }
    __host__ __device__ int size(bool withG) const { return 2 * K + 2 + (withG ? K * K : 0); }
};

constexpr int MAX_PEERS = 16;
struct PeerCfg {
    int nranks = 1, rank = 0;
    double* inbox[MAX_PEERS] = {nullptr};
    unsigned long long* flags[MAX_PEERS] = {nullptr};
    unsigned long long* seq = nullptr;
};

struct LoopState {
    int done;
    int status;
    int success;
    int iterations, nr_iterations, sci_iterations;
    int maxiter, min_sc_iter;
    int haveNr;
    int cholFail;
    double tol, gamma;
    double max_delta, max_diff, gnorm;
    double gn_sci, gn_nr;
};

enum { ROW_C, ROW_GEN_F, ROW_HESS_C, ROW_LOGW_F, ROW_C2, DC_ROWS, ROW_F = DC_ROWS, ROW_POLL, HF_ROWS };

}

struct mbar_b200_ctx {
    int device = 0;
    int K = 0;
    int64_t N = 0;
    int64_t nTiles = 0;
    bool ready = false;
    int kernelChoice = MBAR_B200_KERNEL_AUTO;
    int smCount = 132;

    std::vector<double> h_Nk;
    std::vector<double> h_logNk;
    std::vector<double> h_logNkEff;
    double* d_NkEff = nullptr;
    std::vector<double> h_urowmin;
    std::vector<double> h_uclamp;
    std::vector<double> h_ufar;
    int* d_urowmin = nullptr;
    unsigned long long* d_urowfar = nullptr;
    std::vector<int> active;
    int firstActive = 0;
    double N_total_states = 0;

    double* d_u = nullptr;
    size_t uBytes = 0;
    double* d_xshift = nullptr;
    double* d_wgt = nullptr;
    double* d_sqrtw = nullptr;
    double sumW = 0.0;
    double sumXw = 0.0;
    double sumX = 0.0;
    double* d_c = nullptr;
    double* d_Nk = nullptr;
    unsigned long long* d_rowmask = nullptr;
    unsigned long long* d_zeromask = nullptr;
    unsigned long long* d_onesmask = nullptr;
    double* d_partial = nullptr;
    double* d_out = nullptr;
    double* h_out = nullptr;
    double* d_L = nullptr;
    double* d_W = nullptr;
    unsigned int* d_ticket = nullptr;
    int* d_flag = nullptr;
    double* d_f = nullptr;
    double* h_f = nullptr;
    double* d_scratch = nullptr;
    cudaStream_t stream = nullptr;
    cudaStream_t copyStream = nullptr;
    cudaEvent_t evA = nullptr, evB = nullptr;
    cudaEvent_t evCopy[2] = {nullptr, nullptr};
    double* stage_pinned[2] = {nullptr, nullptr};
    double* stage_dev[2] = {nullptr, nullptr};
    int64_t stageCols = 0;

    double* d_inbox = nullptr;
    mbar::PeerCfg peer;
    bool peerReady = false;
    std::vector<void*> peerMapped;

    void* comm = nullptr;
    int nranks = 1, rank = 0;

    mbar::LoopState* d_loop = nullptr;
    mbar::LoopState* h_loop = nullptr;
    double* d_av = nullptr;
    double* d_outM = nullptr;
    double* d_A = nullptr;
    int* d_active = nullptr;
    unsigned long long* d_seq = nullptr;
    int loopMode = 0;
    int loopBatch = 4;
    int64_t loopPolls = 0;
    bool capturing = false;
    bool graphWarm = false;
    cudaGraphExec_t loopGraph = nullptr;
    std::vector<uint64_t> loopGraphKey;
    int64_t graphLaunches = 0, graphCaptures = 0;
    double* d_Wt = nullptr;
    bool wtAllocFailed = false;
    size_t gpartBytes = 0;
    char lastKernel[200] = "";
    char lastHessKernel[200] = "";
    double lastHessMs = 0.0, lastWeightsMs = 0.0;
    double lastBinMs = 0.0;
    int lastBinChunks = 0;
    double lastRepMs = 0.0;
    int lastRepBatches = 0;
    int64_t lastRepExps = 0;
    cudaEvent_t evH0 = nullptr, evH1 = nullptr, evH2 = nullptr;

    int64_t launches = 0, passes = 0, h2dBytes = 0, d2hBytes = 0;
    double lastPassMs = 0.0;
    double lastLoopMs = 0.0, lastLoopKernelMs = 0.0;
    int lastLoopIters = 0;
    bool timePasses = true;

    double* dc(int row) const { return d_c + (size_t)row * K; }
    double* hf(int row) const { return h_f + (size_t)row * K; }
};

namespace mbar {

struct FusedParams {
    const double* u;
    const double* c;
    const double* c2;
    double* out2;
    double mid2;
    int M;
    const unsigned long long* rowmask;
    const unsigned long long* sampledmask;
    const double* Nk;
    double* partial;
    double* out;
    unsigned int* ticket;
    double* Lout;
    double* Wout;
    const double* wgt;
    double sumW;
    double* f;
    double* cnext;
    PeerCfg peer;
    LoopState* loop;
    int epi, first;
    int64_t N, nTiles, nStages;
    double mid;
    double logFloorN;
    int K, Wk, Wn, Rw, TPW, NS, CW, batch, debugSkip, mode, CL, Kh, allStates;
    uint32_t tileBytes, stageBytes;
};

struct PassWant {
    bool L = false;
    bool unsampled = false;
    bool G = false;
    bool Gall = false;
};

struct NvtxRange {
    explicit NvtxRange(const char* name);
    ~NvtxRange();
};

void host_parallel(int nTasks, const std::function<void(int)>& fn);
int host_parallel_width();

int gpu_numa_node(int device);
struct NumaPrefer {
    bool active = false;
    explicit NumaPrefer(int device);
    ~NumaPrefer();
};

int check_range(mbar_b200_ctx* c, const double* f);
int run_pass(mbar_b200_ctx* c, const double* f, PassWant want);
double global_sumx(mbar_b200_ctx* c, int* rc);
int retile_chunk(mbar_b200_ctx* ctx, const double* d_rowmajor, int64_t ldCols, int64_t tile0,
                 int64_t nTilesChunk, int64_t validCols, cudaStream_t s);
int launch_pass_generic(mbar_b200_ctx* ctx, const double* h_f, bool wantL, bool logAll);
int launch_pass_fused(mbar_b200_ctx* ctx, const double* h_f, bool wantL, bool allStates, bool* usedOut,
                      bool wantW = false, bool* wroteW = nullptr);
int fused_prepare(mbar_b200_ctx* ctx, const double* h_f, bool wantL, bool allStates, FusedParams* out, bool* ok,
                  double* d_cdst = nullptr, double* h_stage = nullptr, bool wantW = false, int M = 1,
                  double midQuantum = 0.0);
int fused_enqueue(mbar_b200_ctx* ctx, const FusedParams& p);
bool fused_applicable(const mbar_b200_ctx* ctx, const double* h_f, bool allStates, double* midOut, double* spreadOut);
int launch_hessian(mbar_b200_ctx* ctx, const double* h_f, bool allRows, bool weightsReady = false);
int launch_hessian_dev(mbar_b200_ctx* ctx, const double* d_ch, bool allRows, LoopState* loop,
                       bool weightsReady = false);
bool ensure_weight_buffer(mbar_b200_ctx* ctx);
int launch_logw(mbar_b200_ctx* ctx, const double* h_f, double* logW_host, int64_t ld, int expo, int64_t n0,
                int64_t n);
int launch_synth(mbar_b200_ctx* ctx, const mbar_b200_synth* spec);
int launch_untile(mbar_b200_ctx* ctx, int64_t n0, int64_t n, double* d_dst, int64_t ld);
int comm_allreduce(mbar_b200_ctx* ctx, double* d_buf, int count, int op );
int agree_row_minima(mbar_b200_ctx* ctx);
int check_unsampled_clamp(const mbar_b200_ctx* ctx);
int reduce_sumx(mbar_b200_ctx* ctx);
int reduce_sumxw(mbar_b200_ctx* ctx);
int set_weights(mbar_b200_ctx* ctx, const double* w_host);
int probe_exp_launch(int which, int64_t n, const double* d_a, double* d_out);

#ifdef __CUDACC__
static __device__ const double MBAR_EXP_TABLE[MBAR_EXP_NT] = {MBAR_EXP_TABLE_VALUES};
__device__ __forceinline__ uint32_t smem_u32(const void* p) {
    return static_cast<uint32_t>(__cvta_generic_to_shared(p));
}
__device__ __forceinline__ void mbar_init(uint32_t bar, uint32_t count) {
    asm volatile("mbarrier.init.shared::cta.b64 [%0], %1;" ::"r"(bar), "r"(count));
}
__device__ __forceinline__ void mbar_fence_init() {
    asm volatile("fence.mbarrier_init.release.cluster;" ::: "memory");
}
__device__ __forceinline__ void mbar_arrive_expect_tx(uint32_t bar, uint32_t bytes) {
    asm volatile("mbarrier.arrive.expect_tx.shared::cta.b64 _, [%0], %1;" ::"r"(bar), "r"(bytes)
                 : "memory");
}
__device__ __forceinline__ void mbar_arrive(uint32_t bar) {
    asm volatile("mbarrier.arrive.shared::cta.b64 _, [%0];" ::"r"(bar) : "memory");
}
__device__ __forceinline__ void mbar_wait(uint32_t bar, uint32_t parity) {
    uint32_t done;
    do {
        asm volatile(
            "{\n\t.reg .pred p;\n\t"
            "mbarrier.try_wait.parity.shared::cta.b64 p, [%1], %2;\n\t"
            "selp.u32 %0, 1, 0, p;\n\t}"
            : "=r"(done)
            : "r"(bar), "r"(parity)
            : "memory");
    } while (!done);
}
__device__ __forceinline__ void mbar_wait_backoff(uint32_t bar, uint32_t parity) {
    uint32_t done;
    for (;;) {
        asm volatile(
            "{\n\t.reg .pred p;\n\t"
            "mbarrier.try_wait.parity.shared::cta.b64 p, [%1], %2, %3;\n\t"
            "selp.u32 %0, 1, 0, p;\n\t}"
            : "=r"(done)
            : "r"(bar), "r"(parity), "r"(0x989680u)
            : "memory");
        if (done) break;
        __nanosleep(200);
    }
}
__device__ __forceinline__ void bulk_g2s(uint32_t dst, const void* src, uint32_t bytes, uint32_t bar) {
    asm volatile(
        "cp.async.bulk.shared::cluster.global.mbarrier::complete_tx::bytes [%0], [%1], %2, [%3];" ::"r"(dst),
        "l"(src), "r"(bytes), "r"(bar)
        : "memory");
}
__device__ __forceinline__ void fence_proxy_async_smem() {
    asm volatile("fence.proxy.async.shared::cta;" ::: "memory");
}
__device__ __forceinline__ void named_bar_sync(int id, int nthreads) {
    asm volatile("bar.sync %0, %1;" ::"r"(id), "r"(nthreads) : "memory");
}

constexpr double EXP_MAGIC = 6755399441055744.0;

__device__ __forceinline__ void exp_split(double a, const double* __restrict__ tab, double& v, int& q) {
    const double t = fma(a, MBAR_EXP_SCALE, EXP_MAGIC);
    const int n = __double2loint(t);
    const double nf = t - EXP_MAGIC;
    const double r = fma(nf, -MBAR_EXP_LN2N, a);
    double p = fma(MBAR_EXP_C5, r, MBAR_EXP_C4);
    p = fma(p, r, MBAR_EXP_C3);
    p = fma(p, r, MBAR_EXP_C2);
    p = fma(p, r, MBAR_EXP_C1);
    p = p * r;
    const double T = tab[n & (MBAR_EXP_NT - 1)];
    v = fma(T, p, T);
    q = n >> 5;
}
__device__ __forceinline__ double scale2(double v, int q) {
    q = max(q, -1021);
    const int hi = __double2hiint(v) + (q << 20);
    return __hiloint2double(hi, __double2loint(v));
}
__device__ __forceinline__ double exp_fast(double a, const double* __restrict__ tab) {
    double v;
    int q;
    exp_split(a, tab, v, q);
    return scale2(v, q);
}
__device__ __forceinline__ double warp_sum(double x) {
#pragma unroll
    for (int o = 16; o > 0; o >>= 1) x += __shfl_xor_sync(0xffffffffu, x, o);
    return x;
}
#endif

__host__ __device__ __forceinline__ double rel_change(double a, double b, double ref, double thr) {
    double div = fabs(ref);
    if (div < thr) div = 1.0;
    return fabs(a - b) / div;
}

inline bool event_ms(cudaEvent_t a, cudaEvent_t b, float* ms) {
    if (cudaEventElapsedTime(ms, a, b) == cudaSuccess) return true;
    cudaGetLastError();
    return false;
}

inline size_t scratch_rendezvous(int K) { return (size_t)K * K + 4 * (size_t)K; }


int open_device(int device, cudaDeviceProp* prop);

template <class T>
int dev_alloc(T** p, size_t count, const char* who) {
    const cudaError_t e = cudaMalloc((void**)p, (count > 0 ? count : 1) * sizeof(T));
    if (e == cudaSuccess) return MBAR_B200_OK;
    *p = nullptr;
    cudaGetLastError();
    set_error("%s: cannot allocate %zu bytes", who, count * sizeof(T));
    return e == cudaErrorMemoryAllocation ? MBAR_B200_ERR_NOMEM : MBAR_B200_ERR_CUDA;
}

struct CallBuffers {
    const char* who;
    std::vector<void*> ptrs;
    explicit CallBuffers(const char* who_) : who(who_) {}
    CallBuffers(const CallBuffers&) = delete;
    CallBuffers& operator=(const CallBuffers&) = delete;
    ~CallBuffers() {
        for (void* p : ptrs) cudaFree(p);
    }
    template <class T>
    int alloc(T** p, size_t count) {
        MBAR_TRY(dev_alloc(p, count, who));
        ptrs.push_back((void*)*p);
        return MBAR_B200_OK;
    }
};

template <class T>
// ... 84 lines not shown
```

pymbar_b200/csrc/loops.cu:

```cuda
#include <nvtx3/nvToolsExt.h>

#include <algorithm>
#include <cmath>
#include <cstdlib>
#include <cstring>
#include <vector>

#include "internal.cuh"

namespace mbar {

NvtxRange::NvtxRange(const char* name) { nvtxRangePushA(name); }
NvtxRange::~NvtxRange() { nvtxRangePop(); }

enum { AV_FSCI = 0, AV_FNR = 1, AV_G = 2, AV_CSCI = 3, AV_CNR = 4, AV_CH = 5, AV_X = 6, AV_DIAG = 7 };

__device__ __forceinline__ bool loop_done(const LoopState* loop) {
    return *reinterpret_cast<const volatile int*>(&loop->done) != 0;
}
__device__ __forceinline__ bool row_on(const unsigned long long* __restrict__ mask, int k) {
    return (mask[k >> 6] >> (k & 63)) & 1ull;
}

__device__ double block_sum(double v, double* s_buf) {
// ... 439 lines not shown
    for (int k : c->active) cur[k] -= f[c->firstActive];
    int rc = MBAR_B200_OK;
    for (int it = 0; it < maxiter; ++it) {
        rc = run_pass(c, cur.data(), PassWant{});
        if (rc != MBAR_B200_OK) break;
        r.passes++;
        sci_step(c, cur, nxt);
        r.max_delta = rel_delta(c, nxt, cur, tol);
        cur.swap(nxt);
        r.iterations = it + 1;
        r.sci_iterations = it + 1;
        if (std::isnan(r.max_delta) || r.max_delta < tol) {
            r.success = 1;
            break;
        }
    }
    if (rc == MBAR_B200_OK) rc = final_gnorm(c, cur, &r);
    r.device_ms = timer.stop();
    if (rc == MBAR_B200_OK) std::memcpy(f, cur.data(), K * sizeof(double));
    if (res) *res = r;
    return rc;
}

static int solve_adaptive_stepped(mbar_b200_ctx* c, double* f, double tol, int32_t maxiter, int32_t min_sc_iter,
                                  double gamma, mbar_b200_solve_result* res) {
    const int K = c->K;
    const PassLayout lay{K};
    const int na = (int)c->active.size();
    std::vector<double> cur(f, f + K), f_sci(K), f_nr(K), g(K, 0.0), g_sci(K), g_nr(K);
    std::vector<double> A, rhs;
    mbar_b200_solve_result r{};
    Events timer;
    MBAR_TRY(timer.start(c->stream));
    for (int k : c->active) cur[k] -= f[c->firstActive];
    int rc = MBAR_B200_OK;
    auto grad_from_out = [&](std::vector<double>& out) {
        double gn = 0.0;
        for (int k = 0; k < K; ++k) {
            out[k] = c->h_Nk[k] > 0 ? c->h_Nk[k] * (c->h_out[k] - 1.0) : 0.0;
            gn += out[k] * out[k];
        }
        return gn;
    };
    for (int it = 0; it < maxiter && rc == MBAR_B200_OK; ++it) {
        PassWant w;
        w.G = true;
        rc = run_pass(c, cur.data(), w);
        if (rc != MBAR_B200_OK) break;
        r.passes++;
        r.hessian_passes++;
        grad_from_out(g);
        sci_step(c, cur, f_sci);
        bool haveNr = false;
        if (na > 1) {
            const int n = na - 1;
            const double* Gh = c->h_out + lay.G();
            double ridge = 0.0, ridgeRel = 0.0, tr = 0.0;
            for (int a = 1; a < na; ++a) {
                const int i = c->active[a];
                tr += c->h_Nk[i] * c->h_out[i];
            }
            for (int attempt = 0; attempt < 4 && !haveNr; ++attempt) {
                A.assign((size_t)n * n, 0.0);
                for (int a = 1; a < na; ++a) {
                    const int i = c->active[a];
                    for (int b = 1; b <= a; ++b) {
                        const int j = c->active[b];
                        double v = -Gh[(size_t)i * K + j];
                        if (i == j) v += c->h_Nk[i] * c->h_out[i] + ridge;
                        A[(size_t)(a - 1) * n + (b - 1)] = v;
                    }
                }
                if (cholesky(A, n)) {
                    rhs.resize(n);
                    for (int a = 1; a < na; ++a) rhs[a - 1] = g[c->active[a]];
                    chol_solve(A, n, rhs);
                    f_nr = cur;
                    for (int a = 1; a < na; ++a) f_nr[c->active[a]] = cur[c->active[a]] - gamma * rhs[a - 1];
                    haveNr = true;
                    for (int a = 1; a < na; ++a)
                        if (!std::isfinite(f_nr[c->active[a]]) || std::fabs(f_nr[c->active[a]]) > 0.5 * C_RANGE)
                            haveNr = false;
                } else {
                    ridgeRel = (ridgeRel == 0.0) ? 1e-12 : ridgeRel * 1e3;
                    ridge = ridgeRel * (tr / n + 1e-300);
                }
            }
        }
        rc = run_pass(c, f_sci.data(), PassWant{});
        if (rc != MBAR_B200_OK) break;
        r.passes++;
        const double gn_sci = grad_from_out(g_sci);
        double gn_nr = INFINITY;
        if (haveNr) {
            rc = run_pass(c, f_nr.data(), PassWant{});
            if (rc != MBAR_B200_OK) break;
            r.passes++;
            gn_nr = grad_from_out(g_nr);
            if (std::isnan(gn_nr)) gn_nr = INFINITY;
        } else {
            f_nr = f_sci;
        }
        std::vector<double> f_old = cur;
        if (gn_sci < gn_nr || r.sci_iterations < min_sc_iter) {
            cur = f_sci;
            r.sci_iterations++;
            r.gnorm = std::sqrt(gn_sci);
        } else {
            cur = f_nr;
            r.nr_iterations++;
            r.gnorm = std::sqrt(gn_nr);
        }
        r.iterations = it + 1;
        r.max_delta = rel_delta(c, cur, f_old, tol);
        double max_diff = 0.0;
        const double thr = std::min(1e-8, tol);
        for (size_t i = 1; i < c->active.size(); ++i) {
            const int k = c->active[i];
            max_diff = std::max(max_diff, rel_change(f_sci[k], f_nr[k], cur[k], thr));
        }
        if (std::isnan(r.max_delta) || (r.max_delta < tol && max_diff < std::sqrt(tol))) {
            r.success = 1;
            break;
        }
    }
    r.device_ms = timer.stop();
    if (rc == MBAR_B200_OK) std::memcpy(f, cur.data(), K * sizeof(double));
    if (res) *res = r;
    return rc;
}

static int sci_iterate_stepped(mbar_b200_ctx* c, double* f, int iters) {
    std::vector<double> cur(f, f + c->K);
    for (int it = 0; it < iters; ++it) {
        MBAR_TRY(run_pass(c, cur.data(), PassWant{}));
        sci_step(c, cur, cur);
    }
    std::memcpy(f, cur.data(), c->K * sizeof(double));
    return MBAR_B200_OK;
}

static int enqueue_sci(mbar_b200_ctx* c, FusedParams p, bool inKernel, int n, LoopState* loop,
                       const cudaEvent_t* ev) {
    const int K = c->K;
    p.loop = loop;
    p.first = c->firstActive;
    if (inKernel) {
        p.epi = 1;
        p.f = c->d_f;
        p.cnext = c->dc(ROW_C);
        if (c->peerReady) p.peer = c->peer;
    }
    for (int it = 0; it < n; ++it) {
        if (ev) MBAR_CUDA(cudaEventRecord(ev[2 * it], c->stream));
        MBAR_TRY(fused_enqueue(c, p));
        if (ev) MBAR_CUDA(cudaEventRecord(ev[2 * it + 1], c->stream));
        if (!inKernel) {
            MBAR_TRY(comm_allreduce(c, c->d_out, K + 2, 0));
            sci_loop_epilogue_kernel<<<1, 256, 0, c->stream>>>(c->d_out, c->d_f, c->dc(ROW_C), c->d_Nk, c->d_rowmask,
                                                               K, p.first, p.mid, loop);
            c->launches++;
        }
    }
    return MBAR_B200_OK;
}

static int poll_batches(mbar_b200_ctx* c, std::vector<double>& cur, int* itersBefore, bool* fallback,
                        const std::function<int(const double*, bool*)>& batch) {
    const int K = c->K;
    *fallback = false;
    for (;;) {
        *itersBefore = c->h_loop->iterations;
        bool ok = false;
        MBAR_TRY(batch(cur.data(), &ok));
        if (!ok) {
            *fallback = true;
            return MBAR_B200_OK;
        }
        MBAR_CUDA(cudaMemcpyAsync(c->h_loop, c->d_loop, sizeof(LoopState), cudaMemcpyDeviceToHost, c->stream));
        MBAR_CUDA(cudaMemcpyAsync(c->hf(ROW_POLL), c->d_f, (size_t)K * sizeof(double), cudaMemcpyDeviceToHost,
                                  c->stream));
        MBAR_CUDA(cudaStreamSynchronize(c->stream));
        c->d2hBytes += (int64_t)K * 8 + (int64_t)sizeof(LoopState);
        c->loopPolls++;
        MBAR_CUDA(cudaGetLastError());
        const LoopState& st = *c->h_loop;
        if (st.status != 0) {
            MBAR_REQUIRE(st.status != 2, MBAR_B200_ERR_COMM,
                         "peer exchange timed out inside the pass kernel (a rank did not arrive)");
            *fallback = true;
            return MBAR_B200_OK;
        }
        std::memcpy(cur.data(), c->hf(ROW_POLL), K * sizeof(double));
        if (st.done) return MBAR_B200_OK;
    }
}

static int solve_sci_device(mbar_b200_ctx* c, double* f, double tol, int32_t maxiter, mbar_b200_solve_result* res) {
    MBAR_REQUIRE(c->ready, MBAR_B200_ERR_NOT_READY, "u_kn has not been uploaded");
    MBAR_CUDA(cudaSetDevice(c->device));
    MBAR_TRY(check_range(c, f));
    if (!device_loop_possible(c) || maxiter < 1 || c->active.size() < 2)
        return solve_sci_stepped(c, f, tol, maxiter, res);
    std::vector<double> cur(f, f + c->K);
    for (int k : c->active) cur[k] -= f[c->firstActive];
    Events timer;
    MBAR_TRY(timer.start(c->stream));
    MBAR_TRY(loop_begin(c, tol, maxiter, 0, 1.0));
    const bool inKernel = sci_epilogue_in_kernel(c);
    if (c->peerReady && inKernel) MBAR_TRY(comm_rendezvous(c));
    int itersBefore = 0;
    bool fallback = false;
    MBAR_TRY(poll_batches(c, cur, &itersBefore, &fallback, [&](const double* fb, bool* ok) -> int {
        FusedParams p;
        MBAR_TRY(fused_prepare(c, fb, false, false, &p, ok));
        if (!*ok) return MBAR_B200_OK;
        MBAR_TRY(upload_f(c, fb));
        return enqueue_sci(c, p, inKernel, c->loopBatch, c->d_loop, nullptr);
    }));
    mbar_b200_solve_result r{};
    int rc;
    if (fallback) {
        rc = solve_sci_stepped(c, cur.data(), tol, std::max(maxiter - itersBefore, 1), &r);
        r.iterations += itersBefore;
        r.sci_iterations += itersBefore;
        r.passes += itersBefore;
    } else {
        const LoopState& st = *c->h_loop;
        r.iterations = r.sci_iterations = st.iterations;
        r.passes = st.iterations;
        r.success = st.success;
        r.max_delta = st.max_delta;
        rc = final_gnorm(c, cur, &r);
    }
    r.device_ms = timer.stop();
    if (rc == MBAR_B200_OK)
        for (int k : c->active) f[k] = cur[k];
    if (res) *res = r;
    return rc;
}

static int enqueue_adaptive_iteration(mbar_b200_ctx* c, const FusedParams& pF, const FusedParams& pS,
                                      const FusedParams& pN, const FusedParams* pM) {
    const int K = c->K;
    const PassLayout lay{K};
    const int na = (int)c->active.size();
    const int n = na - 1;
    const int g0 = c->firstActive;
    const bool nccl = c->nranks > 1 && !c->peerReady;
    double* av = c->d_av;
    MBAR_TRY(fused_enqueue(c, pF));
    if (nccl) MBAR_TRY(comm_allreduce(c, c->d_out, K + 2, 0));
    adapt_pre_kernel<<<1, 256, 0, c->stream>>>(c->d_out, c->d_f, c->d_Nk, c->d_rowmask, K, g0, pF.mid, av, c->d_loop);
    MBAR_TRY(launch_hessian_dev(c, av + AV_CH * K, false, c->d_loop, pF.Wout != nullptr));
    if (c->nranks > 1) MBAR_TRY(comm_allreduce(c, c->d_out + lay.G(), K * K, 0));
    const bool smem = (size_t)n * n * 8 + 2 * ((size_t)n + 2) * 8 <= 200 * 1024;
    const size_t shBytes = 2 * ((size_t)n + 2) * 8 + (smem ? (size_t)n * n * 8 : 0);
    auto kern = smem ? newton_kernel<true> : newton_kernel<false>;
    static size_t attr[16][2] = {{0}};
    size_t& a = attr[c->device & 15][smem ? 0 : 1];
    if (a < shBytes) {
        MBAR_CUDA(cudaFuncSetAttribute(kern, cudaFuncAttributeMaxDynamicSharedMemorySize, (int)shBytes));
        a = shBytes;
    }
    const int bgrid = (int)std::min<int64_t>(((int64_t)n * n + 255) / 256, 4 * c->smCount);
    const int nthreads = n >= 96 ? 1024 : n >= 32 ? 512 : 256;
    for (int attempt = 0; attempt < 2; ++attempt) {
        newton_build_kernel<<<bgrid, 256, 0, c->stream>>>(c->d_out + lay.G(), av, c->d_active, na, K, c->d_A,
                                                         attempt ? 1.0e-10 : 0.0, attempt, c->d_loop);
        kern<<<1, nthreads, shBytes, c->stream>>>(c->d_A, na, K, c->d_active, c->d_f, c->d_Nk, av, pF.mid, attempt,
                                                 attempt == 1, c->d_loop);
    }
    MBAR_CUDA(cudaGetLastError());
    if (pM) {
        MBAR_TRY(fused_enqueue(c, *pM));
        if (nccl) {
            MBAR_TRY(comm_allreduce(c, pM->out, K + 2, 0));
            MBAR_TRY(comm_allreduce(c, pM->out2, K + 2, 0));
        }
    } else {
        MBAR_TRY(fused_enqueue(c, pS));
        if (nccl) MBAR_TRY(comm_allreduce(c, pS.out, K + 2, 0));
        MBAR_TRY(fused_enqueue(c, pN));
        if (nccl) MBAR_TRY(comm_allreduce(c, pN.out, K + 2, 0));
    }
    adapt_post_kernel<<<1, 256, 0, c->stream>>>(pS.out, pN.out, av, c->d_f, c->dc(ROW_C), c->d_Nk, c->d_rowmask, K, g0,
                                               pF.mid, c->d_loop);
    MBAR_CUDA(cudaGetLastError());
    c->launches += 6;
    return MBAR_B200_OK;
}

static void key_push(std::vector<uint64_t>& key, const FusedParams& p) {
    auto bits = [](double v) { uint64_t u; std::memcpy(&u, &v, 8); return u; };
    const uint64_t f[] = {(uint64_t)(uintptr_t)p.u, (uint64_t)(uintptr_t)p.c, (uint64_t)(uintptr_t)p.c2,
                          (uint64_t)(uintptr_t)p.out, (uint64_t)(uintptr_t)p.out2, (uint64_t)(uintptr_t)p.Lout,
                          (uint64_t)(uintptr_t)p.Wout, (uint64_t)(uintptr_t)p.wgt, (uint64_t)(uintptr_t)p.loop,
                          (uint64_t)(uintptr_t)p.rowmask, (uint64_t)(uintptr_t)p.Nk, (uint64_t)(uintptr_t)p.peer.seq,
                          bits(p.mid), bits(p.mid2), bits(p.sumW), (uint64_t)p.N, (uint64_t)p.nStages,
                          (uint64_t)p.K | ((uint64_t)p.CL << 16) | ((uint64_t)p.M << 24) | ((uint64_t)p.mode << 28) |
                              ((uint64_t)p.NS << 32) | ((uint64_t)p.TPW << 40) | ((uint64_t)p.Wk << 48) | ((uint64_t)p.Rw << 56),
                          (uint64_t)p.peer.nranks | ((uint64_t)p.peer.rank << 8) | ((uint64_t)p.epi << 16) |
                              ((uint64_t)p.first << 24) | ((uint64_t)p.debugSkip << 56)};
    key.insert(key.end(), f, f + sizeof(f) / sizeof(f[0]));
}

static int run_adaptive_batch(mbar_b200_ctx* c, const FusedParams& pF, const FusedParams& pS, const FusedParams& pN,
                              const FusedParams* pM, int batch) {
    static const bool noGraph = std::getenv("MBAR_B200_NO_GRAPH") != nullptr;
    static const bool graphMulti = std::getenv("MBAR_B200_GRAPH_MULTI") != nullptr;
    if (noGraph || !c->graphWarm || (c->nranks > 1 && !graphMulti)) {
        for (int b = 0; b < batch; ++b) MBAR_TRY(enqueue_adaptive_iteration(c, pF, pS, pN, pM));
        c->graphWarm = true;
        return MBAR_B200_OK;
    }
    std::vector<uint64_t> key;
    key_push(key, pF);
    key_push(key, pS);
    key_push(key, pN);
    if (pM) key_push(key, *pM);
    key.push_back((uint64_t)c->nranks | ((uint64_t)c->peerReady << 8) | ((uint64_t)(uintptr_t)c->comm << 16));
    if (!c->loopGraph || key != c->loopGraphKey) {
        if (c->loopGraph) {
            cudaGraphExecDestroy(c->loopGraph);
            c->loopGraph = nullptr;
        }
        const int64_t launches0 = c->launches, passes0 = c->passes;
        c->capturing = true;
        cudaError_t e = cudaStreamBeginCapture(c->stream, cudaStreamCaptureModeRelaxed);
        int rc = MBAR_B200_OK;
        if (e == cudaSuccess) rc = enqueue_adaptive_iteration(c, pF, pS, pN, pM);
        cudaGraph_t g = nullptr;
        if (e == cudaSuccess) e = cudaStreamEndCapture(c->stream, &g);
        c->capturing = false;
        c->launches = launches0;
        c->passes = passes0;
        if (e == cudaSuccess && rc == MBAR_B200_OK && g) e = cudaGraphInstantiate(&c->loopGraph, g, 0);
        if (g) cudaGraphDestroy(g);
        if (e != cudaSuccess || rc != MBAR_B200_OK || !c->loopGraph) {
            cudaGetLastError();
            c->loopGraph = nullptr;
            c->loopGraphKey.clear();
            for (int b = 0; b < batch; ++b) MBAR_TRY(enqueue_adaptive_iteration(c, pF, pS, pN, pM));
            return MBAR_B200_OK;
        }
        c->loopGraphKey = key;
        c->graphCaptures++;
    }
    for (int b = 0; b < batch; ++b) {
        MBAR_CUDA(cudaGraphLaunch(c->loopGraph, c->stream));
        c->graphLaunches++;
        c->launches += 11;
        c->passes += pM ? 3 : 4;
    }
    return MBAR_B200_OK;
}

static int solve_adaptive_device(mbar_b200_ctx* c, double* f, double tol, int32_t maxiter, int32_t min_sc_iter,
                                 double gamma, mbar_b200_solve_result* res) {
    MBAR_REQUIRE(c->ready, MBAR_B200_ERR_NOT_READY, "u_kn has not been uploaded");
    MBAR_CUDA(cudaSetDevice(c->device));
    MBAR_TRY(check_range(c, f));
    const int K = c->K;
    if (!device_loop_possible(c) || maxiter < 1 || c->active.size() < 2)
        return solve_adaptive_stepped(c, f, tol, maxiter, min_sc_iter, gamma, res);
    std::vector<double> cur(f, f + K);
    for (int k : c->active) cur[k] -= f[c->firstActive];
    Events timer;
    MBAR_TRY(timer.start(c->stream));
    MBAR_TRY(loop_begin(c, tol, maxiter, min_sc_iter, gamma));
    if (c->peerReady) MBAR_TRY(comm_rendezvous(c));
    bool usedM2 = false;
    int itersBefore = 0;
    bool fallback = false;
    MBAR_TRY(poll_batches(c, cur, &itersBefore, &fallback, [&](const double* fb, bool* ok) -> int {
        FusedParams pF;
        MBAR_TRY(fused_prepare(c, fb, true, false, &pF, ok, nullptr, nullptr, true, 1, 16.0));
        if (!*ok) return MBAR_B200_OK;
        MBAR_TRY(upload_f(c, fb));
        pF.loop = c->d_loop;
        pF.first = c->firstActive;
        if (c->peerReady) pF.peer = c->peer;
        FusedParams pS = pF, pN = pF;
        pS.Wout = pN.Wout = nullptr;
        pS.c = c->d_av + AV_CSCI * K;
        pS.out = c->d_outM;
        pS.Lout = nullptr;
        pN.c = c->d_av + AV_CNR * K;
        pN.out = c->d_outM + PassLayout{K}.size(false);
        pN.Lout = nullptr;
        FusedParams pM;
        bool okM = false;
        static const bool noM2 = std::getenv("MBAR_B200_NO_M2") != nullptr;
        if (!noM2)
            MBAR_TRY(fused_prepare(c, fb, false, false, &pM, &okM, c->d_av + AV_CSCI * K, c->hf(ROW_C2), false, 2,
                                   16.0));
        if (okM) {
            pM.loop = c->d_loop;
            pM.first = c->firstActive;
            if (c->peerReady) pM.peer = c->peer;
            pM.c = c->d_av + AV_CSCI * K;
            pM.c2 = c->d_av + AV_CNR * K;
            pM.mid2 = pM.mid;
            pM.out = pS.out;
            pM.out2 = pN.out;
        }
        usedM2 = usedM2 || okM;
        return run_adaptive_batch(c, pF, pS, pN, okM ? &pM : nullptr, c->loopBatch);
    }));
    const int passesPerIter = usedM2 ? 2 : 3;
    const LoopState st = *c->h_loop;
    mbar_b200_solve_result r{};
    int rc = MBAR_B200_OK;
    if (fallback) {
        const int msi = std::max(min_sc_iter - st.sci_iterations, 0);
        rc = solve_adaptive_stepped(c, cur.data(), tol, std::max(maxiter - itersBefore, 1), msi, gamma, &r);
        r.iterations += itersBefore;
        r.passes += passesPerIter * itersBefore;
        r.hessian_passes += itersBefore;
    } else {
        r.iterations = st.iterations;
        r.nr_iterations = st.nr_iterations;
        r.sci_iterations = st.sci_iterations;
        r.passes = passesPerIter * st.iterations;
        r.hessian_passes = st.iterations;
        r.success = st.success;
        r.max_delta = st.max_delta;
        r.gnorm = st.gnorm;
    }
    r.device_ms = timer.stop();
    if (rc == MBAR_B200_OK)
        for (int k : c->active) f[k] = cur[k];
    if (res) *res = r;
    return rc;
}

}

using namespace mbar;

extern "C" {

int mbar_b200_solve_sci(mbar_b200_ctx* c, double* f, double tol, int32_t maxiter, mbar_b200_solve_result* res) {
    MBAR_REQUIRE(c && f, MBAR_B200_ERR_INVALID, "NULL argument");
    NvtxRange nvtx_("mbar_b200::solve_sci");
    if (c->loopMode == 1) return solve_sci_stepped(c, f, tol, maxiter, res);
    return solve_sci_device(c, f, tol, maxiter, res);
}

int mbar_b200_solve_adaptive(mbar_b200_ctx* c, double* f, double tol, int32_t maxiter, int32_t min_sc_iter,
                             double gamma, mbar_b200_solve_result* res) {
    MBAR_REQUIRE(c && f, MBAR_B200_ERR_INVALID, "NULL argument");
    NvtxRange nvtx_("mbar_b200::solve_adaptive");
    if (c->loopMode == 1) return solve_adaptive_stepped(c, f, tol, maxiter, min_sc_iter, gamma, res);
    return solve_adaptive_device(c, f, tol, maxiter, min_sc_iter, gamma, res);
}

int mbar_b200_set_loop_mode(mbar_b200_ctx* c, int32_t mode, int32_t batch) {
    MBAR_REQUIRE(c, MBAR_B200_ERR_INVALID, "ctx is NULL");
    MBAR_REQUIRE(mode == 0 || mode == 1, MBAR_B200_ERR_INVALID, "mode=%d (0 device-resident, 1 host-stepped)", mode);
    c->loopMode = mode;
    if (batch >= 1) c->loopBatch = batch > 64 ? 64 : batch;
    return MBAR_B200_OK;
}

int mbar_b200_get_loop_stats(const mbar_b200_ctx* c, int64_t* polls, int32_t* mode, int32_t* batch) {
    MBAR_REQUIRE(c, MBAR_B200_ERR_INVALID, "ctx is NULL");
    if (polls) *polls = c->loopPolls;
    if (mode) *mode = c->loopMode;
    if (batch) *batch = c->loopBatch;
    return MBAR_B200_OK;
}

int mbar_b200_get_graph_stats(const mbar_b200_ctx* c, int64_t* captures, int64_t* launches) {
    MBAR_REQUIRE(c, MBAR_B200_ERR_INVALID, "ctx is NULL");
    if (captures) *captures = c->graphCaptures;
    if (launches) *launches = c->graphLaunches;
    return MBAR_B200_OK;
}

int mbar_b200_sci_iterate(mbar_b200_ctx* c, double* f, int32_t iters) {
    MBAR_REQUIRE(c && f && iters >= 0, MBAR_B200_ERR_INVALID, "bad argument");
    MBAR_REQUIRE(c->ready, MBAR_B200_ERR_NOT_READY, "u_kn has not been uploaded");
    MBAR_CUDA(cudaSetDevice(c->device));
    MBAR_TRY(check_range(c, f));
    const int K = c->K;
    FusedParams p;
    bool ok = false;
    if (c->kernelChoice != MBAR_B200_KERNEL_GENERIC) MBAR_TRY(fused_prepare(c, f, false, false, &p, &ok));
    if (!ok) return sci_iterate_stepped(c, f, iters);
    MBAR_TRY(upload_f(c, f));
    Events ev;
    const bool perLaunch = c->timePasses && iters > 0 && iters <= 4096;
    if (perLaunch) MBAR_TRY(ev.create(2 * (size_t)iters));
    Events timer;
    MBAR_TRY(timer.start(c->stream));
    const bool inKernel = sci_epilogue_in_kernel(c);
    MBAR_REQUIRE(c->nranks == 1 || c->comm, MBAR_B200_ERR_NOT_READY,
                 "sharded problem (%d ranks) without a communicator: call mbar_b200_comm_init", c->nranks);
    if (inKernel && c->peerReady) MBAR_TRY(comm_rendezvous(c));
    NvtxRange nvtx_("mbar_b200::sci_iterate");
    MBAR_TRY(enqueue_sci(c, p, inKernel, iters, nullptr, perLaunch ? ev.ev.data() : nullptr));
    c->lastLoopMs = timer.stop();
    double ksum = 0.0;
    for (int it = 0; perLaunch && it < iters; ++it) ksum += ev.ms(2 * it, 2 * it + 1);
    c->lastLoopKernelMs = ksum;
    c->lastLoopIters = iters;
    MBAR_CUDA(cudaGetLastError());
    double* fh = c->hf(ROW_F);
    MBAR_CUDA(cudaMemcpyAsync(fh, c->d_f, K * sizeof(double), cudaMemcpyDeviceToHost, c->stream));
    const PassLayout lay{K};
    MBAR_CUDA(cudaMemcpyAsync(c->h_out, c->d_out, (size_t)lay.size(false) * sizeof(double),
                              cudaMemcpyDeviceToHost, c->stream));
    MBAR_CUDA(cudaStreamSynchronize(c->stream));
    c->d2hBytes += K * 8 + lay.size(false) * 8;
    float ms = 0.f;
    if (event_ms(c->evA, c->evB, &ms)) c->lastPassMs = ms;
    MBAR_REQUIRE(!(iters > 0 && c->h_out[lay.flag()] >= 1.0e6), MBAR_B200_ERR_COMM,
                 "peer exchange timed out inside the pass kernel (a rank did not arrive)");
    if (p.debugSkip) return MBAR_B200_OK;
    if (iters > 0 && c->h_out[lay.flag()] != 0.0) fh[c->firstActive] = NAN;
    bool finite = true;
    for (int k : c->active) finite = finite && std::isfinite(fh[k]);
    if (!finite) return sci_iterate_stepped(c, f, iters);
    for (int k = 0; k < K; ++k)
        if (c->h_Nk[k] > 0) f[k] = fh[k];
    return MBAR_B200_OK;
}

int mbar_b200_last_loop_ms(mbar_b200_ctx* c, double* total_ms, double* kernel_ms_sum, int32_t* iters) {
    MBAR_REQUIRE(c, MBAR_B200_ERR_INVALID, "ctx is NULL");
    if (total_ms) *total_ms = c->lastLoopMs;
    if (kernel_ms_sum) *kernel_ms_sum = c->lastLoopKernelMs;
    if (iters) *iters = c->lastLoopIters;
    return MBAR_B200_OK;
}

}
```

pymbar_b200/csrc/pass_fused.cu:

```cuda
#include <cmath>
#include <cstdlib>

#include "internal.cuh"

namespace mbar {


__host__ __device__ constexpr int fused_slots(int CL) { return CL > 1 ? CL * 8 : 16; }
constexpr uint32_t FUSED_COPY_CHUNK = 32768;

__host__ __device__ inline size_t fused_smem_header(int K, int CL, int M = 1) {
    size_t b = 256 + (size_t)M * (((size_t)K + 32) * 8 + 2 * (size_t)fused_slots(CL) * 32 * 8 + 256 * 8 + 128 + 128) +
               64 + 64;
    return (b + 127) & ~(size_t)127;
}

__device__ __forceinline__ double lds_f64(const double* p) {
    double v;
    asm volatile("ld.shared.f64 %0, [%1];" : "=d"(v) : "r"(smem_u32(p)));
    return v;
}

struct TabRef {
    int hi, lo;
    uint32_t laneBase;
};

template <int R, int B, int R0, bool PREFETCH, int MODE, bool MASKED>
__device__ __forceinline__ void exp_batch(const double (&cu)[B], const double (&uu)[B], const TabRef tr,
                                          double (&e)[R], double& Dp, const double* nextC,
                                          const double* nextU, double (&cn)[B], double (&un)[B],
                                          uint32_t actbits) {
    constexpr bool LDSTAB = MODE & 1, ETRICK = MODE & 2;
    double t[B], r[B], pl[B], T[B];
#pragma unroll
    for (int i = 0; i < B; ++i) {
        if (ETRICK) {
            r[i] = uu[i];
            t[i] = fma(uu[i], -MBAR_EXP_SCALE, EXP_MAGIC);
        } else {
            r[i] = cu[i] - uu[i];
            t[i] = fma(r[i], MBAR_EXP_SCALE, EXP_MAGIC);
        }
    }
#pragma unroll
    for (int i = 0; i < B; ++i) {
        const int n = __double2loint(t[i]);
        if (LDSTAB) {
            const uint32_t addr = (((uint32_t)n << 8) & 0x1f00u) | tr.laneBase;
            asm volatile("ld.shared.f64 %0, [%1];" : "=d"(T[i]) : "r"(addr));
        } else {
            T[i] = __hiloint2double(__shfl_sync(0xffffffffu, tr.hi, n), __shfl_sync(0xffffffffu, tr.lo, n));
        }
    }
    if (PREFETCH) {
#pragma unroll
        for (int i = 0; i < B; ++i) un[i] = lds_f64(nextU + i * TILE_N);
#pragma unroll
        for (int i = 0; i < B; i += 2) {
            double2 c2;
            asm volatile("ld.shared.v2.f64 {%0, %1}, [%2];" : "=d"(c2.x), "=d"(c2.y) : "r"(smem_u32(nextC + i)));
            cn[i] = c2.x;
            cn[i + 1] = c2.y;
        }
    }
    if (ETRICK) {
#pragma unroll
        for (int i = 0; i < B; ++i) r[i] = fma(t[i] - EXP_MAGIC, MBAR_EXP_LN2N, r[i]);
#pragma unroll
        for (int i = 0; i < B; ++i) pl[i] = fma(-MBAR_EXP_C5, r[i], MBAR_EXP_C4);
#pragma unroll
        for (int i = 0; i < B; ++i) pl[i] = fma(pl[i], r[i], -MBAR_EXP_C3);
#pragma unroll
        for (int i = 0; i < B; ++i) pl[i] = fma(pl[i], r[i], MBAR_EXP_C2);
#pragma unroll
        for (int i = 0; i < B; ++i) pl[i] = fma(pl[i], r[i], -MBAR_EXP_C1);
    } else {
#pragma unroll
        for (int i = 0; i < B; ++i) r[i] = fma(t[i] - EXP_MAGIC, -MBAR_EXP_LN2N, r[i]);
#pragma unroll
        for (int i = 0; i < B; ++i) pl[i] = fma(MBAR_EXP_C5, r[i], MBAR_EXP_C4);
#pragma unroll
        for (int i = 0; i < B; ++i) pl[i] = fma(pl[i], r[i], MBAR_EXP_C3);
#pragma unroll
        for (int i = 0; i < B; ++i) pl[i] = fma(pl[i], r[i], MBAR_EXP_C2);
#pragma unroll
        for (int i = 0; i < B; ++i) pl[i] = fma(pl[i], r[i], MBAR_EXP_C1);
    }
#pragma unroll
    for (int i = 0; i < B; ++i) pl[i] = pl[i] * r[i];
#pragma unroll
    for (int i = 0; i < B; ++i) {
        e[R0 + i] = scale2(fma(T[i], pl[i], T[i]), __double2loint(t[i]) >> 5);
        if (MASKED && !((actbits >> (R0 + i)) & 1u)) e[R0 + i] = 0.0;
        if (ETRICK)
            Dp = fma(cu[i], e[R0 + i], Dp);
        else
            Dp += e[R0 + i];
    }
}

template <int R, int B, int R0, int MODE, bool MASKED>
__device__ __forceinline__ void exp_rows(double (&cA)[B], double (&uA)[B], double (&cB)[B], double (&uB)[B],
                                         const TabRef tr, double (&e)[R], double& Dp,
                                         const double* cbase, const double* ubase, uint32_t actbits) {
    if constexpr (R0 + B < R) {
        exp_batch<R, B, R0, true, MODE, MASKED>(cA, uA, tr, e, Dp, cbase + R0 + B,
                                                ubase + (R0 + B) * TILE_N, cB, uB, actbits);
        exp_rows<R, B, R0 + B, MODE, MASKED>(cB, uB, cA, uA, tr, e, Dp, cbase, ubase, actbits);
    } else {
        exp_batch<R, B, R0, false, MODE, MASKED>(cA, uA, tr, e, Dp, nullptr, nullptr, cB, uB, actbits);
    }
}

__device__ __forceinline__ void logprod_push(double D, double& mprod, int& esum) {
    const int hi = __double2hiint(D);
    esum += (hi >> 20) - 1023;
    mprod *= __hiloint2double((hi & 0x000fffff) | 0x3ff00000, __double2loint(D));
}
__device__ __forceinline__ void logprod_renorm(double& mprod, int& esum) {
    const int hi = __double2hiint(mprod);
    esum += (hi >> 20) - 1023;
    mprod = __hiloint2double((hi & 0x000fffff) | 0x3ff00000, __double2loint(mprod));
}

__device__ __forceinline__ unsigned cluster_ctarank() {
    unsigned r;
    asm volatile("mov.u32 %0, %%cluster_ctarank;" : "=r"(r));
    return r;
}
__device__ __forceinline__ void st_cluster_f64(double* localPtr, unsigned rank, double v) {
    uint32_t ra;
    asm volatile("mapa.shared::cluster.u32 %0, %1, %2;" : "=r"(ra) : "r"(smem_u32(localPtr)), "r"(rank));
    asm volatile("st.shared::cluster.f64 [%0], %1;" ::"r"(ra), "d"(v) : "memory");
}
__device__ __forceinline__ void cluster_barrier() {
    asm volatile("barrier.cluster.arrive.release.aligned;\n\tbarrier.cluster.wait.acquire.aligned;" ::: "memory");
}

template <int R, bool FULL, int CW, int BATCH, int MODE, int CL, bool WST = false, int M = 1>
__global__ void __launch_bounds__(CW * 32, 1) pass_fused_kernel(const FusedParams p) {
    static_assert(M == 1 || ((MODE & 2) && R <= 16 && !WST), "M = 2 needs the multiplicative constant and R <= 16");
    extern __shared__ __align__(128) unsigned char smem_raw[];
    if (p.loop && *reinterpret_cast<volatile int*>(&p.loop->done)) return;
    const int K = p.K;
    const int half = (CL > 1) ? (int)cluster_ctarank() : 0;
    const int kbase = (CL > 1) ? half * p.Kh : 0;
    const int Kl = (CL > 1) ? max(0, min(p.Kh, K - kbase)) : K;
    const unsigned nGroups = gridDim.x / CL, grp = blockIdx.x / CL;
    double* tab = reinterpret_cast<double*>(smem_raw);
    double* c_s = tab + 32;
    double* c_s2 = c_s + (K + 32);
    double* xD = c_s + M * (K + 32);
    constexpr int SLOTS = fused_slots(CL);
    double* sred = xD + 2 * M * SLOTS * 32;
    double* s_sumL = sred + M * 256;
    int* s_bad = reinterpret_cast<int*>(s_sumL + M * 16);
    uint64_t* bar_full = reinterpret_cast<uint64_t*>(s_sumL + M * 32);
    uint64_t* bar_empty = bar_full + 8;
    unsigned char* stages = smem_raw + fused_smem_header(K, CL, M);
    __shared__ bool s_last;

    const int lane = threadIdx.x & 31, warp = threadIdx.x >> 5;
    if (threadIdx.x < 32) tab[threadIdx.x] = MBAR_EXP_TABLE[threadIdx.x];
    for (int k = threadIdx.x; k < Kl; k += blockDim.x)
        c_s[k] = (MODE & 2) ? exp(p.c[kbase + k]) : p.c[kbase + k];
    for (int i = threadIdx.x; i < 32; i += blockDim.x) c_s[Kl + i] = 0.0;
    if constexpr (M == 2) {
        for (int k = threadIdx.x; k < Kl; k += blockDim.x) c_s2[k] = exp(p.c2[kbase + k]);
        for (int i = threadIdx.x; i < 32; i += blockDim.x) c_s2[Kl + i] = 0.0;
    }
    for (int i = threadIdx.x; i < 2 * M * SLOTS * 32; i += blockDim.x) xD[i] = 0.0;
    const uint32_t tabRep = (smem_u32(stages + (size_t)p.NS * p.stageBytes) + 8191u) & ~8191u;
    if (MODE & 1)
        for (int i = threadIdx.x; i < 32 * 32; i += blockDim.x)
            asm volatile("st.shared.f64 [%0], %1;" ::"r"(tabRep + i * 8), "d"(MBAR_EXP_TABLE[i >> 5]));
    if (threadIdx.x == 0) {
        for (int i = 0; i < p.NS; ++i) {
            mbar_init(smem_u32(&bar_full[i]), 1);
            mbar_init(smem_u32(&bar_empty[i]), CW);
        }
        mbar_fence_init();
    }
    __syncthreads();
    if (CL > 1) cluster_barrier();

    const int tilesPerStage = p.Wn * p.TPW;
    double acc[R];
    double acc2[M == 2 ? R : 1];
#pragma unroll
    for (int r = 0; r < R; ++r) acc[r] = 0.0;
#pragma unroll
    for (int r = 0; r < (M == 2 ? R : 1); ++r) acc2[r] = 0.0;
    double sumL = 0.0, sumL2 = 0.0;
    int bad = 0, bad2 = 0;
    const int g = warp / p.Wk, w = warp % p.Wk;
    const int k0 = w * p.Rw;

    auto issue = [&](int it2, int slot2, int wrap2) {
        const int64_t s2 = (int64_t)grp + (int64_t)it2 * nGroups;
        if (s2 >= p.nStages) return;
        if (wrap2 > 0) mbar_wait(smem_u32(&bar_empty[slot2]), (wrap2 - 1) & 1);
        const int64_t tile0 = s2 * tilesPerStage;
        const int64_t ntl = min((int64_t)tilesPerStage, p.nTiles - tile0);
        const uint32_t fb = smem_u32(&bar_full[slot2]);
        const uint32_t dst = smem_u32(stages + (size_t)slot2 * p.stageBytes);
        if (Kl <= 0) {
            mbar_arrive_expect_tx(fb, 0);
        } else if (CL == 1) {
            const uint32_t bytes = (uint32_t)ntl * p.tileBytes;
            mbar_arrive_expect_tx(fb, bytes);
            const unsigned char* src =
                reinterpret_cast<const unsigned char*>(p.u) + (size_t)tile0 * p.tileBytes;
            for (uint32_t off = 0; off < bytes; off += FUSED_COPY_CHUNK)
                bulk_g2s(dst + off, src + off, min(FUSED_COPY_CHUNK, bytes - off), fb);
        } else {
            const uint32_t tb = (uint32_t)Kl * TILE_N * 8;
            mbar_arrive_expect_tx(fb, (uint32_t)ntl * tb);
            for (int64_t t = 0; t < ntl; ++t)
                bulk_g2s(dst + (uint32_t)t * tb,
                         reinterpret_cast<const unsigned char*>(p.u) + (size_t)(tile0 + t) * p.tileBytes +
                             (size_t)kbase * TILE_N * 8,
                         tb, fb);
        }
    };
    if (threadIdx.x == 0)
        for (int i = 0; i < p.NS - 1; ++i) issue(i, i, 0);
    {
        uint32_t actbits = 0;
#pragma unroll
        for (int r = 0; r < R; ++r) {
            const int k = kbase + k0 + r;
            if (r < p.Rw && k0 + r < Kl && ((p.rowmask[k >> 6] >> (k & 63)) & 1ull)) actbits |= 1u << r;
        }
        int par = 0;
        int it = 0;
        double mprod = 1.0;
        int esum = 0, npush = 0;
        double mprod2 = 1.0;
        int esum2 = 0;
        TabRef tr;
        tr.hi = __double2hiint(MBAR_EXP_TABLE[lane]);
        tr.lo = __double2loint(MBAR_EXP_TABLE[lane]);
        tr.laneBase = tabRep + lane * 8;
        int slot = 0, wrap = 0;
        int pslot = p.NS - 1, pwrap = 0;
        for (int64_t s = grp; s < p.nStages; s += nGroups, ++it) {
            if (threadIdx.x == 0) issue(it + p.NS - 1, pslot, pwrap);
            if (++pslot == p.NS) { pslot = 0; ++pwrap; }
            mbar_wait(smem_u32(&bar_full[slot]), wrap & 1);
            const double* sb = reinterpret_cast<const double*>(stages + (size_t)slot * p.stageBytes);
            for (int j = 0; j < p.TPW; ++j) {
                if (p.debugSkip) break;
                const int tis = j * p.Wn + g;
                const int64_t tile = s * tilesPerStage + tis;
                if (tile >= p.nTiles) break;
                const double* tp = sb + ((size_t)tis * Kl + k0) * TILE_N + lane;
                const double wn = (!FULL && p.wgt) ? __ldg(p.wgt + tile * TILE_N + lane) : 1.0;
                double e[R];
                double Dp = 0.0;
                {
                    constexpr int B = R < BATCH ? R : BATCH;
                    double cA[B], uA[B], cB[B], uB[B];
#pragma unroll
                    for (int i = 0; i < B; ++i) {
                        uA[i] = lds_f64(tp + i * TILE_N);
                        cA[i] = lds_f64(c_s + k0 + i);
                    }
                    exp_rows<R, B, 0, MODE, !FULL>(cA, uA, cB, uB, tr, e, Dp, c_s + k0, tp, actbits);
                }
                double D = Dp, D2 = 0.0, Dp2 = 0.0;
                if constexpr (M == 2) {
#pragma unroll
                    for (int r = 0; r < R; ++r) Dp2 = fma(lds_f64(c_s2 + k0 + r), e[r], Dp2);
                    D2 = Dp2;
                }
                if (CL >= 4) {
                    double* xb = xD + par * M * SLOTS * 32 + lane;
                    xb[(CL + w) * 32] = Dp;
                    if constexpr (M == 2) xb[(SLOTS + CL + w) * 32] = Dp2;
                    named_bar_sync(1, CW * 32);
                    if (w == 0) {
                        double s1 = 0.0, s2 = 0.0;
#pragma unroll
                        for (int ww = 0; ww < 8; ++ww) s1 += xb[(CL + ww) * 32];
                        if constexpr (M == 2) {
#pragma unroll
                            for (int ww = 0; ww < 8; ++ww) s2 += xb[(SLOTS + CL + ww) * 32];
                        }
                        double* x = xb + half * 32;
                        *x = s1;
                        if constexpr (M == 2) x[SLOTS * 32] = s2;
#pragma unroll
                        for (int q = 1; q < CL; ++q) {
                            st_cluster_f64(x, (unsigned)((half + q) % CL), s1);
                            if constexpr (M == 2) st_cluster_f64(x + SLOTS * 32, (unsigned)((half + q) % CL), s2);
                        }
                    }
                    cluster_barrier();
                    D = 0.0;
#pragma unroll
                    for (int q = 0; q < CL; ++q) D += xb[q * 32];
                    if constexpr (M == 2) {
                        D2 = 0.0;
#pragma unroll
                        for (int q = 0; q < CL; ++q) D2 += xb[(SLOTS + q) * 32];
                    }
                    par ^= 1;
                } else if (CL > 1) {
                    double* x = xD + (par * M * SLOTS + half * 8 + w) * 32 + lane;
                    *x = Dp;
                    if constexpr (M == 2) x[SLOTS * 32] = Dp2;
#pragma unroll
                    for (int q = 1; q < CL; ++q) {
                        st_cluster_f64(x, (unsigned)((half + q) % CL), Dp);
                        if constexpr (M == 2) st_cluster_f64(x + SLOTS * 32, (unsigned)((half + q) % CL), Dp2);
                    }
                    cluster_barrier();
                    const double* xs = xD + par * M * SLOTS * 32 + lane;
                    D = 0.0;
#pragma unroll
                    for (int ww = 0; ww < CL * 8; ++ww) D += xs[ww * 32];
                    if constexpr (M == 2) {
                        D2 = 0.0;
#pragma unroll
                        for (int ww = 0; ww < CL * 8; ++ww) D2 += xs[(SLOTS + ww) * 32];
                    }
                    par ^= 1;
                } else if (p.Wk > 1) {
                    double* x = xD + (par * M * SLOTS + g * p.Wk) * 32 + lane;
                    x[w * 32] = Dp;
                    if constexpr (M == 2) x[(SLOTS + w) * 32] = Dp2;
                    named_bar_sync(1 + g, p.Wk * 32);
                    D = 0.0;
                    for (int ww = 0; ww < p.Wk; ++ww) D += x[ww * 32];
                    if constexpr (M == 2) {
                        D2 = 0.0;
                        for (int ww = 0; ww < p.Wk; ++ww) D2 += x[(SLOTS + ww) * 32];
                    }
                    par ^= 1;
                }
                const bool valid = tile * TILE_N + lane < p.N;
                if (valid && !(D > 1e-250 && D < 1e250)) bad = 1;
                const double rD = 1.0 / D;
                const double invD = valid ? (FULL ? rD : rD * wn) : 0.0;
#pragma unroll
                for (int r = 0; r < R; ++r) acc[r] = fma(e[r], invD, acc[r]);
                if constexpr (M == 2) {
                    if (valid && !(D2 > 1e-250 && D2 < 1e250)) bad2 = 1;
                    const double rD2 = 1.0 / D2;
                    const double invD2 = valid ? (FULL ? rD2 : rD2 * wn) : 0.0;
#pragma unroll
                    for (int r = 0; r < R; ++r) acc2[r] = fma(e[r], invD2, acc2[r]);
                }
                if (WST) {
                    const double inv0 = valid ? ((!FULL && p.wgt) ? rD * sqrt(wn) : rD) : 0.0;
                    double* wp = p.Wout + ((size_t)tile * K + kbase + k0) * TILE_N;
#pragma unroll
                    for (int r = 0; r < R; ++r) {
                        if (FULL || (r < p.Rw && k0 + r < Kl)) {
                            double wv = e[r] * inv0;
                            if (MODE & 2) wv *= lds_f64(c_s + k0 + r);
                            const int k = kbase + k0 + r;
                            wp[r * TILE_N + (lane ^ ((k & 7) << 2))] = wv;
                        }
                    }
                }
                if (w == 0 && half == 0) {
                    if (valid) {
                        if (!FULL && p.wgt) {
                            sumL += wn * log(D);
                            if constexpr (M == 2) sumL2 += wn * log(D2);
                        } else {
                            logprod_push(D, mprod, esum);
                            if constexpr (M == 2) logprod_push(D2, mprod2, esum2);
                            if ((++npush & 255) == 0) {
                                logprod_renorm(mprod, esum);
                                if constexpr (M == 2) logprod_renorm(mprod2, esum2);
                            }
                        }
                    }
                    if (p.Lout) p.Lout[tile * TILE_N + lane] = log(D) + p.mid;
                }
            }
            __syncwarp();
            if (lane == 0) mbar_arrive(smem_u32(&bar_empty[slot]));
            if (++slot == p.NS) { slot = 0; ++wrap; }
        }
#pragma unroll
        for (int r = 0; r < R; ++r) {
            const double t = warp_sum(acc[r]);
            if (lane == 0 && r < p.Rw && k0 + r < Kl) sred[g * Kl + k0 + r] = t;
        }
        sumL += (double)esum * 0.693147180559945309417232 + log(mprod);
        sumL = warp_sum(sumL);
        bad = __any_sync(0xffffffffu, bad);
        if (lane == 0) {
            s_sumL[warp] = (w == 0 && half == 0) ? sumL : 0.0;
            s_bad[warp] = bad;
        }
        if constexpr (M == 2) {
#pragma unroll
            for (int r = 0; r < R; ++r) {
                const double t = warp_sum(acc2[r]);
                if (lane == 0 && r < p.Rw && k0 + r < Kl) sred[256 + g * Kl + k0 + r] = t;
            }
            sumL2 += (double)esum2 * 0.693147180559945309417232 + log(mprod2);
            sumL2 = warp_sum(sumL2);
            bad2 = __any_sync(0xffffffffu, bad2);
            if (lane == 0) {
                s_sumL[16 + warp] = (w == 0 && half == 0) ? sumL2 : 0.0;
                s_bad[32 + warp] = bad2;
            }
        }
    }
    if (CL > 1) cluster_barrier();
    __syncthreads();

    constexpr int PW = M;
    double* P = p.partial + (size_t)grp * (PW * (K + 2));
    for (int k = threadIdx.x; k < Kl; k += blockDim.x) {
        double t = 0.0;
// ... 195 lines not shown
                    L->done = 1;
                } else if (m < L->tol) {
                    L->success = 1;
                    L->done = 1;
                } else if (it >= L->maxiter) {
                    L->done = 1;
                }
            }
        }
    }
}

static int fused_mode(double spread) {
    int mode = 3;
    if (const char* v = std::getenv("MBAR_B200_FUSED_MODE")) mode = std::atoi(v) & 3;
    mode |= 1;
    if (spread > 600.0) mode &= 1;
    return mode;
}

bool fused_applicable(const mbar_b200_ctx* ctx, const double* h_f, bool allStates, double* midOut,
                      double* spreadOut) {
    if (ctx->K > 2048) return false;
    double lo = INFINITY, hi = -INFINITY;
    for (int k = 0; k < ctx->K; ++k) {
        if (!allStates && !(ctx->h_Nk[k] > 0)) continue;
        const double c = h_f[k] + ctx->h_logNkEff[k];
        if (!std::isfinite(c)) return false;
        lo = std::fmin(lo, c);
        hi = std::fmax(hi, c);
    }
    if (hi - lo >= FUSED_SPREAD) return false;
    if (std::fabs(hi) > C_RANGE || std::fabs(lo) > C_RANGE) return false;
    if (allStates) {
        const bool mult = fused_mode(hi - lo) & 2;
        const double mid = 0.5 * (hi + lo);
        for (int k = 0; k < ctx->K; ++k) {
            if (ctx->h_Nk[k] > 0) continue;
            const double arg = (mult ? 0.0 : h_f[k] + ctx->h_logNkEff[k] - mid) - ctx->h_urowmin[k];
            if (arg > FUSED_MAX_ARG) return false;
        }
    }
    if (midOut) *midOut = 0.5 * (hi + lo);
    if (spreadOut) *spreadOut = hi - lo;
    return true;
}

int fused_prepare(mbar_b200_ctx* ctx, const double* h_f, bool wantL, bool allStates, FusedParams* out,
                  bool* ok, double* d_cdst, double* h_stage, bool wantW, int M, double midQuantum) {
    if (!d_cdst) d_cdst = ctx->dc(ROW_C);
    if (!h_stage) h_stage = ctx->hf(ROW_C);
    *ok = false;
    double mid = 0.0, spread = 0.0;
    if (!fused_applicable(ctx, h_f, allStates, &mid, &spread)) return MBAR_B200_OK;
    if (midQuantum > 0.0) mid = midQuantum * std::nearbyint(mid / midQuantum);
    const int K = ctx->K;
    FusedParams p{};
    p.K = K;
    const int mode = fused_mode(spread);
    p.logFloorN = LOG_FLOOR_S + std::log(ctx->N_total_states);
    p.allStates = allStates ? 1 : 0;
    p.M = M;
    if (M == 2 && (!(mode & 2) || K > 1024 || K < 2 || allStates || wantW)) return MBAR_B200_OK;
    if (M == 2 && K > 128 && !std::getenv("MBAR_B200_M2_CLUSTERS")) return MBAR_B200_OK;
    const int cw = 8;
    const int rmax = (M == 2) ? 16 : 32;
    const int perCta = cw * rmax;
    p.CL = K > 4 * perCta ? 8 : K > 2 * perCta ? 4 : K > perCta ? 2 : 1;
    p.Kh = (K + p.CL - 1) / p.CL;
    if (p.CL > 1) p.Kh = (p.Kh + 1) & ~1;
    int wk = 1;
    while (wk * rmax < p.Kh) wk *= 2;
    p.Wk = wk;
    p.CW = cw;
    p.batch = 8;
    p.mode = mode;
    p.debugSkip = std::getenv("MBAR_B200_FUSED_SKIP") ? 1 : 0;
    p.Wn = cw / p.Wk;
    p.Rw = (p.Kh + p.Wk - 1) / p.Wk;
    p.Rw = (p.Rw + 1) & ~1;
    p.tileBytes = (uint32_t)K * TILE_N * 8;
    const uint32_t ctaTileBytes = (uint32_t)p.Kh * TILE_N * 8;
    int tpw = (int)(65536u / (p.Wn * ctaTileBytes));
    p.TPW = tpw < 1 ? 1 : (tpw > 8 ? 8 : tpw);
    p.stageBytes = (uint32_t)p.Wn * p.TPW * ctaTileBytes;
    {
        const int rt = p.Rw <= 8 ? 8 : p.Rw <= 16 ? 16 : p.Rw <= 24 ? 24 : 32;
        const int over = (p.Wk - 1) * p.Rw + rt - p.Kh;
        if (over > 0) p.stageBytes += (uint32_t)over * TILE_N * 8;
        p.stageBytes = (p.stageBytes + 127u) & ~127u;
    }
    const size_t header = fused_smem_header(K, p.CL, M);
    int ns = (int)((225 * 1024 - header - 16384) / p.stageBytes);
    while (ns < 2 && p.TPW > 1) {
        const uint32_t pad = p.stageBytes - (uint32_t)p.Wn * p.TPW * ctaTileBytes;
        p.TPW /= 2;
        p.stageBytes = (((uint32_t)p.Wn * p.TPW * ctaTileBytes + pad) + 127u) & ~127u;
        ns = (int)((225 * 1024 - header - 16384) / p.stageBytes);
    }
    p.NS = ns > 8 ? 8 : ns;
    if (p.NS < 2) return MBAR_B200_OK;
    const int tilesPerStage = p.Wn * p.TPW;
    p.nStages = (ctx->nTiles + tilesPerStage - 1) / tilesPerStage;
    p.N = ctx->N;
    p.nTiles = ctx->nTiles;
    p.mid = mid;
    p.u = ctx->d_u;
    p.c = d_cdst;
    p.rowmask = allStates ? ctx->d_onesmask : ctx->d_rowmask;
    p.sampledmask = ctx->d_rowmask;
    p.Nk = allStates ? ctx->d_NkEff : ctx->d_Nk;
    p.partial = ctx->d_partial;
    p.out = ctx->d_out;
    p.ticket = ctx->d_ticket;
    if (wantL && !ctx->d_L)
        MBAR_CUDA(cudaMalloc((void**)&ctx->d_L, (size_t)ctx->nTiles * TILE_N * sizeof(double)));
    p.Lout = wantL ? ctx->d_L : nullptr;
    p.Wout = (wantW && !allStates && M == 1 && ensure_weight_buffer(ctx)) ? ctx->d_Wt : nullptr;
    p.wgt = ctx->d_wgt;
    p.sumW = ctx->d_wgt ? ctx->sumW : (double)ctx->N;
    for (int k = 0; k < K; ++k)
        h_stage[k] = (!allStates && std::isinf(ctx->h_logNk[k])) ? 0.0 : h_f[k] + ctx->h_logNkEff[k] - mid;
    MBAR_CUDA(cudaMemcpyAsync(d_cdst, h_stage, (size_t)K * sizeof(double), cudaMemcpyHostToDevice,
                              ctx->stream));
    ctx->h2dBytes += K * 8;
    *out = p;
    *ok = true;
    return MBAR_B200_OK;
}

int fused_enqueue(mbar_b200_ctx* ctx, const FusedParams& p) {
    const size_t smem = fused_smem_header(p.K, p.CL, p.M) + (size_t)p.NS * p.stageBytes + 16384;
    int64_t grid = p.nStages < ctx->smCount / p.CL ? p.nStages : ctx->smCount / p.CL;
    grid *= p.CL;
    const int Rt = p.Rw <= 8 ? 8 : p.Rw <= 16 ? 16 : (p.Rw <= 24 && p.M == 1) ? 24 : 32;
    const bool full = (p.Rw == Rt) && (p.K == p.CL * p.Wk * p.Rw) &&
                      ((int)ctx->active.size() == p.K || p.allStates) && !p.wgt;
    void (*kern)(const FusedParams) = nullptr;
    int which = 0;
#define PICK(R_, CL_, ID_)                                                                           \
    if (Rt == R_ && p.CL == CL_) {                                                                   \
        if (!full && !(p.mode & 2)) { kern = pass_fused_kernel<R_, false, 8, 8, 1, CL_>; which = ID_; } \
        else if (!full) { kern = pass_fused_kernel<R_, false, 8, 8, 3, CL_>; which = ID_ + 1; }        \
        else if (!(p.mode & 2)) { kern = pass_fused_kernel<R_, true, 8, 8, 1, CL_>; which = ID_ + 2; } \
        else { kern = pass_fused_kernel<R_, true, 8, 8, 3, CL_>; which = ID_ + 3; }                    \
    }
#define PICKW(R_, CL_, ID_)                                                                          \
    if (Rt == R_ && p.CL == CL_ && p.Wout) {                                                         \
        if (!full && !(p.mode & 2)) { kern = pass_fused_kernel<R_, false, 8, 8, 1, CL_, true>; which = ID_; } \
        else if (!full) { kern = pass_fused_kernel<R_, false, 8, 8, 3, CL_, true>; which = ID_ + 1; }        \
        else if (!(p.mode & 2)) { kern = pass_fused_kernel<R_, true, 8, 8, 1, CL_, true>; which = ID_ + 2; } \
        else { kern = pass_fused_kernel<R_, true, 8, 8, 3, CL_, true>; which = ID_ + 3; }                    \
    }
#define PICKM(R_, CL_, ID_)                                                                          \
    if (Rt == R_ && p.CL == CL_) {                                                                   \
        if (!full) { kern = pass_fused_kernel<R_, false, 8, 8, 3, CL_, false, 2>; which = ID_; }     \
        else { kern = pass_fused_kernel<R_, true, 8, 8, 3, CL_, false, 2>; which = ID_ + 1; }        \
    }
    if (p.M == 2) {
        MBAR_REQUIRE((p.mode & 2) && !p.Wout && p.c2 && p.out2, MBAR_B200_ERR_INVALID, "bad M = 2 launch");
        PICKM(8, 1, 40) PICKM(16, 1, 42) PICKM(16, 2, 44) PICKM(16, 4, 46) PICKM(16, 8, 48)
    } else {
        PICK(8, 1, 0) PICK(16, 1, 4) PICK(32, 1, 8) PICK(32, 2, 12) PICK(32, 4, 16) PICK(32, 8, 20)
        PICK(24, 1, 60) PICK(24, 2, 64) PICK(24, 4, 68) PICK(24, 8, 72)
        PICKW(32, 1, 24) PICKW(32, 2, 28) PICKW(32, 4, 32) PICKW(32, 8, 36) PICKW(16, 1, 52) PICKW(8, 1, 56)
        PICKW(24, 1, 76) PICKW(24, 2, 80) PICKW(24, 4, 84) PICKW(24, 8, 88)
    }
#undef PICKM
#undef PICKW
#undef PICK
    MBAR_REQUIRE(kern, MBAR_B200_ERR_INVALID, "no fused kernel variant for K=%d", p.K);
    const bool isW = (which >= 24 && which < 40) || (which >= 52 && which < 60) || which >= 76;
    MBAR_REQUIRE(!p.Wout || isW, MBAR_B200_ERR_INVALID, "no weight-storing fused variant for K=%d", p.K);
    snprintf(ctx->lastKernel, sizeof(ctx->lastKernel),
             "pass_fused_kernel<R=%d, %s, CW=8, BATCH=8, MODE=%d (%s), CL=%d%s> grid=%lld NS=%d TPW=%d", Rt,
             full ? "FULL" : "MASKED", (p.mode & 2) ? 3 : 1,
             (p.mode & 2) ? "LDS table + multiplicative state constant" : "LDS table", p.CL,
             (which >= 40 && which < 52) ? ", M=2 (two candidates per launch)"
                           : isW ? ", WST (weights stored for the Hessian)" : "",
             (long long)grid, p.NS, p.TPW);
    static size_t attrSetAll[16][96] = {{0}};
    size_t* attrSet = attrSetAll[ctx->device & 15];
    if (attrSet[which] < smem) {
        MBAR_CUDA(cudaFuncSetAttribute(kern, cudaFuncAttributeMaxDynamicSharedMemorySize, (int)smem));
        attrSet[which] = smem;
    }
    if (!ctx->capturing) MBAR_CUDA(cudaEventRecord(ctx->evA, ctx->stream));
    if (p.CL == 1) {
        kern<<<(unsigned)grid, p.CW * 32, smem, ctx->stream>>>(p);
    } else {
        cudaLaunchConfig_t cfg = {};
        cfg.gridDim = dim3((unsigned)grid);
        cfg.blockDim = dim3(p.CW * 32);
        cfg.dynamicSmemBytes = smem;
        cfg.stream = ctx->stream;
        cudaLaunchAttribute at[1];
        at[0].id = cudaLaunchAttributeClusterDimension;
        at[0].val.clusterDim.x = (unsigned)p.CL;
        at[0].val.clusterDim.y = 1;
        at[0].val.clusterDim.z = 1;
        cfg.attrs = at;
        cfg.numAttrs = 1;
        MBAR_CUDA(cudaLaunchKernelEx(&cfg, kern, p));
    }
    if (!ctx->capturing) MBAR_CUDA(cudaEventRecord(ctx->evB, ctx->stream));
    ctx->launches++;
    ctx->passes++;
    MBAR_CUDA(cudaGetLastError());
    return MBAR_B200_OK;
}

int launch_pass_fused(mbar_b200_ctx* ctx, const double* h_f, bool wantL, bool allStates, bool* usedOut,
                      bool wantW, bool* wroteW) {
    FusedParams p;
    if (wroteW) *wroteW = false;
    MBAR_TRY(fused_prepare(ctx, h_f, wantL, allStates, &p, usedOut, nullptr, nullptr, wantW));
    if (!*usedOut) return MBAR_B200_OK;
    if (wroteW) *wroteW = p.Wout != nullptr;
    return fused_enqueue(ctx, p);
}

__global__ void __launch_bounds__(32) probe_exp_kernel(int which, int64_t n, const double* __restrict__ a,
                                                       double* __restrict__ out) {
    __shared__ double tab[MBAR_EXP_NT];
    __shared__ double rep[2 * 32 * 32];
    const int lane = threadIdx.x;
    tab[lane] = MBAR_EXP_TABLE[lane];
    const uint32_t tabRep = (smem_u32(rep) + 8191u) & ~8191u;
    for (int i = lane; i < 32 * 32; i += 32)
        asm volatile("st.shared.f64 [%0], %1;" ::"r"(tabRep + i * 8), "d"(MBAR_EXP_TABLE[i >> 5]));
    __syncwarp();
    TabRef tr;
    tr.hi = __double2hiint(MBAR_EXP_TABLE[lane]);
    tr.lo = __double2loint(MBAR_EXP_TABLE[lane]);
    tr.laneBase = tabRep + lane * 8;
    const int64_t base = (int64_t)blockIdx.x * 256;
    double cu[8], uu[8], e[8], cn[8], un[8], Dp = 0.0;
#pragma unroll
    for (int i = 0; i < 8; ++i) {
        const int64_t j = base + i * 32 + lane;
        const double x = j < n ? a[j] : 0.0;
        cu[i] = which == 1 ? x : 0.0;
        uu[i] = which == 1 ? 0.0 : -x;
        e[i] = which == 0 ? exp_fast(x, tab) : 0.0;
    }
    if (which == 1) exp_batch<8, 8, 0, false, 1, false>(cu, uu, tr, e, Dp, nullptr, nullptr, cn, un, 0u);
    if (which == 2) exp_batch<8, 8, 0, false, 3, false>(cu, uu, tr, e, Dp, nullptr, nullptr, cn, un, 0u);
#pragma unroll
    for (int i = 0; i < 8; ++i) {
        const int64_t j = base + i * 32 + lane;
        if (j < n) out[j] = e[i];
    }
}

int probe_exp_launch(int which, int64_t n, const double* d_a, double* d_out) {
    probe_exp_kernel<<<(unsigned)((n + 255) / 256), 32>>>(which, n, d_a, d_out);
    MBAR_CUDA(cudaGetLastError());
    return MBAR_B200_OK;
}

}
```

Baseline: 391.4 billion.

## Cache exp(-u') on device and reuse it in later fused passes

After the first fused pass, a multiplicative-mode pass writes the per-entry exponentials exp(-u') into a device buffer the same size as u. Later passes run a new E0 kernel variant that streams this buffer instead of u and skips the table-based exp evaluation. The goal is to remove per-iteration exp arithmetic from the inner loop. Costs are a second full-size device allocation, a pass that writes an extra copy of the data, invalidation whenever u is re-uploaded, and little benefit if the kernel is already bound by HBM bandwidth, since the bytes read per pass stay the same.

```diff
diff --git a/pymbar_b200/csrc/api.cu b/pymbar_b200/csrc/api.cu
--- a/pymbar_b200/csrc/api.cu
+++ b/pymbar_b200/csrc/api.cu
@@ -270,6 +270,7 @@
             MBAR_TRY(comm_allreduce(c, p[0].out2, K + 2, 0));
         } else {
             for (int m = 0; m < M; ++m) {
+                e0_select(c, p[m], true);
                 MBAR_TRY(fused_enqueue(c, p[m]));
                 MBAR_TRY(comm_allreduce(c, p[m].out, K + 2, 0));
             }
diff --git a/pymbar_b200/csrc/ctx.cu b/pymbar_b200/csrc/ctx.cu
--- a/pymbar_b200/csrc/ctx.cu
+++ b/pymbar_b200/csrc/ctx.cu
@@ -164,6 +164,14 @@
     slot.ptr = ptr;
     slot.bytes = bytes;
     return old;
+}
+
+static std::vector<mbar_b200_ctx*> g_live;
+static std::mutex g_liveMutex;
+static void release_e0_caches(int device) {
+    std::lock_guard<std::mutex> g(g_liveMutex);
+    for (mbar_b200_ctx* c : g_live)
+        if (device < 0 || c->device == device) e0_release(c);
 }
 
 __device__ __forceinline__ void row_min_push(int* rowMin, double v, int lane) {
@@ -608,6 +616,12 @@
     if (pool_enabled()) {
         c->d_u = static_cast<double*>(pool_take(g_pool[device & 15].u, uBytes));
         if (c->d_u) c->uBytes = 0;
+    }
+    if (!c->d_u && cudaMalloc((void**)&c->d_u, uBytes) != cudaSuccess) {
+        cudaGetLastError();
+        c->d_u = nullptr;
+        release_e0_caches(device);
+        cudaSetDevice(device);
     }
     if (!c->d_u) ALLOC(c->d_u, uBytes);
     ALLOC(c->d_xshift, nPad * sizeof(double));
@@ -677,12 +691,20 @@
     CREATE_CUDA(cudaMemset(c->d_urowmin, 0, 2 * (size_t)K * sizeof(int)));
     CREATE_CUDA(cudaMemset(c->d_urowfar, 0, (size_t)K * sizeof(unsigned long long)));
 #undef CREATE_CUDA
+    {
+        std::lock_guard<std::mutex> g(g_liveMutex);
+        g_live.push_back(c);
+    }
     *out = c;
     return MBAR_B200_OK;
 }
 
 int mbar_b200_destroy(mbar_b200_ctx* c) {
     if (!c) return MBAR_B200_OK;
+    {
+        std::lock_guard<std::mutex> g(g_liveMutex);
+        g_live.erase(std::remove(g_live.begin(), g_live.end(), c), g_live.end());
+    }
     cudaSetDevice(c->device);
     if (c->comm) mbar_b200_comm_destroy(c);
     for (void* pm : c->peerMapped) cudaIpcCloseMemHandle(pm);
@@ -709,7 +731,7 @@
     cudaFree(c->d_W); cudaFree(c->d_ticket); cudaFree(c->d_flag); cudaFree(c->d_urowmin); cudaFree(c->d_urowfar); cudaFree(c->d_f);
     cudaFree(c->d_scratch);
     cudaFree(c->d_loop); cudaFree(c->d_av); cudaFree(c->d_outM); cudaFree(c->d_A); cudaFree(c->d_active);
-    cudaFree(c->d_seq); cudaFree(c->d_Wt);
+    cudaFree(c->d_seq); cudaFree(c->d_Wt); cudaFree(c->d_e0);
     if (c->loopGraph) cudaGraphExecDestroy(c->loopGraph);
     if (c->h_loop) cudaFreeHost(c->h_loop);
     if (c->evH0) cudaEventDestroy(c->evH0);
@@ -734,6 +756,7 @@
 int mbar_b200_trim(void) {
     int cur = 0;
     cudaGetDevice(&cur);
+    release_e0_caches(-1);
     for (int d = 0; d < 16; ++d) {
         DevicePool old;
         {
@@ -867,6 +890,7 @@
     MBAR_REQUIRE(ld >= c->N, MBAR_B200_ERR_INVALID, "ld=%lld < N_local=%lld", (long long)ld,
                  (long long)c->N);
     MBAR_CUDA(cudaSetDevice(c->device));
+    e0_invalidate(c);
     cudaPointerAttributes attr;
     bool pinned = false;
     if (cudaPointerGetAttributes(&attr, u_host) == cudaSuccess)
@@ -1087,6 +1111,7 @@
     MBAR_REQUIRE(ld >= c->N, MBAR_B200_ERR_INVALID, "ld=%lld < N_local", (long long)ld);
     MBAR_CUDA(cudaSetDevice(c->device));
     MBAR_CUDA(cudaDeviceSynchronize());
+    e0_invalidate(c);
     MBAR_TRY(retile_chunk(c, u_dev, ld, 0, c->nTiles, c->N, c->stream));
     return finish_upload(c);
 }
@@ -1094,6 +1119,7 @@
 int mbar_b200_synthesize(mbar_b200_ctx* c, const mbar_b200_synth* spec) {
     MBAR_REQUIRE(c && spec && spec->O_k && spec->k_k, MBAR_B200_ERR_INVALID, "NULL argument");
     MBAR_CUDA(cudaSetDevice(c->device));
+    e0_invalidate(c);
     MBAR_TRY(launch_synth(c, spec));
     MBAR_TRY(reduce_sumx(c));
     MBAR_TRY(reduce_sumxw(c));
diff --git a/pymbar_b200/csrc/hessian.cu b/pymbar_b200/csrc/hessian.cu
--- a/pymbar_b200/csrc/hessian.cu
+++ b/pymbar_b200/csrc/hessian.cu
@@ -534,6 +534,12 @@
     if (cudaMalloc((void**)&ctx->d_Wt, bytes) != cudaSuccess) {
         cudaGetLastError();
         ctx->d_Wt = nullptr;
+        if (ctx->d_e0 && !ctx->capturing) {
+            e0_release(ctx);
+            if (cudaMalloc((void**)&ctx->d_Wt, bytes) == cudaSuccess) return true;
+            cudaGetLastError();
+            ctx->d_Wt = nullptr;
+        }
         ctx->wtAllocFailed = true;
         return false;
     }
diff --git a/pymbar_b200/csrc/internal.cuh b/pymbar_b200/csrc/internal.cuh
--- a/pymbar_b200/csrc/internal.cuh
+++ b/pymbar_b200/csrc/internal.cuh
@@ -158,6 +158,9 @@
     int64_t graphLaunches = 0, graphCaptures = 0;
     double* d_Wt = nullptr;
     bool wtAllocFailed = false;
+    double* d_e0 = nullptr;
+    int e0State = 0;
+    int e0Passes = 0;
     size_t gpartBytes = 0;
     char lastKernel[200] = "";
     char lastHessKernel[200] = "";
@@ -208,7 +211,11 @@
     double logFloorN;
     int K, Wk, Wn, Rw, TPW, NS, CW, batch, debugSkip, mode, CL, Kh, allStates;
     uint32_t tileBytes, stageBytes;
-};
+    double* e0;
+    int e0mode;
+};
+enum { E0_OFF = 0, E0_WRITE = 1, E0_READ = 2 };
+enum { E0_NONE = 0, E0_VALID = 1, E0_NO_ROOM = 2 };
 
 struct PassWant {
     bool L = false;
@@ -244,6 +251,9 @@
                   double* d_cdst = nullptr, double* h_stage = nullptr, bool wantW = false, int M = 1,
                   double midQuantum = 0.0);
 int fused_enqueue(mbar_b200_ctx* ctx, const FusedParams& p);
+void e0_select(mbar_b200_ctx* ctx, FusedParams& p, bool mayWrite);
+void e0_invalidate(mbar_b200_ctx* ctx);
+void e0_release(mbar_b200_ctx* ctx);
 bool fused_applicable(const mbar_b200_ctx* ctx, const double* h_f, bool allStates, double* midOut, double* spreadOut);
 int launch_hessian(mbar_b200_ctx* ctx, const double* h_f, bool allRows, bool weightsReady = false);
 int launch_hessian_dev(mbar_b200_ctx* ctx, const double* d_ch, bool allRows, LoopState* loop,
diff --git a/pymbar_b200/csrc/loops.cu b/pymbar_b200/csrc/loops.cu
--- a/pymbar_b200/csrc/loops.cu
+++ b/pymbar_b200/csrc/loops.cu
@@ -615,6 +615,7 @@
         if (c->peerReady) p.peer = c->peer;
     }
     for (int it = 0; it < n; ++it) {
+        e0_select(c, p, loop == nullptr || it == 0);
         if (ev) MBAR_CUDA(cudaEventRecord(ev[2 * it], c->stream));
         MBAR_TRY(fused_enqueue(c, p));
         if (ev) MBAR_CUDA(cudaEventRecord(ev[2 * it + 1], c->stream));
@@ -764,7 +765,8 @@
                           (uint64_t)p.K | ((uint64_t)p.CL << 16) | ((uint64_t)p.M << 24) | ((uint64_t)p.mode << 28) |
                               ((uint64_t)p.NS << 32) | ((uint64_t)p.TPW << 40) | ((uint64_t)p.Wk << 48) | ((uint64_t)p.Rw << 56),
                           (uint64_t)p.peer.nranks | ((uint64_t)p.peer.rank << 8) | ((uint64_t)p.epi << 16) |
-                              ((uint64_t)p.first << 24) | ((uint64_t)p.debugSkip << 56)};
+                              ((uint64_t)p.first << 24) | ((uint64_t)p.e0mode << 48) | ((uint64_t)p.debugSkip << 56),
+                          (uint64_t)(uintptr_t)p.e0};
     key.insert(key.end(), f, f + sizeof(f) / sizeof(f[0]));
 }
 
@@ -852,6 +854,8 @@
         pN.c = c->d_av + AV_CNR * K;
         pN.out = c->d_outM + PassLayout{K}.size(false);
         pN.Lout = nullptr;
+        e0_select(c, pS, false);
+        e0_select(c, pN, false);
         FusedParams pM;
         bool okM = false;
         static const bool noM2 = std::getenv("MBAR_B200_NO_M2") != nullptr;
diff --git a/pymbar_b200/csrc/pass_fused.cu b/pymbar_b200/csrc/pass_fused.cu
--- a/pymbar_b200/csrc/pass_fused.cu
+++ b/pymbar_b200/csrc/pass_fused.cu
@@ -30,7 +30,7 @@
 __device__ __forceinline__ void exp_batch(const double (&cu)[B], const double (&uu)[B], const TabRef tr,
                                           double (&e)[R], double& Dp, const double* nextC,
                                           const double* nextU, double (&cn)[B], double (&un)[B],
-                                          uint32_t actbits) {
+                                          uint32_t actbits, double* e0w = nullptr, uint32_t wbits = 0u) {
     constexpr bool LDSTAB = MODE & 1, ETRICK = MODE & 2;
     double t[B], r[B], pl[B], T[B];
 #pragma unroll
@@ -90,8 +90,14 @@
 #pragma unroll
     for (int i = 0; i < B; ++i) pl[i] = pl[i] * r[i];
 #pragma unroll
+    for (int i = 0; i < B; ++i) e[R0 + i] = scale2(fma(T[i], pl[i], T[i]), __double2loint(t[i]) >> 5);
+    if (e0w) {
+#pragma unroll
+        for (int i = 0; i < B; ++i)
+            if (!MASKED || ((wbits >> (R0 + i)) & 1u)) e0w[(R0 + i) * TILE_N] = e[R0 + i];
+    }
+#pragma unroll
     for (int i = 0; i < B; ++i) {
-        e[R0 + i] = scale2(fma(T[i], pl[i], T[i]), __double2loint(t[i]) >> 5);
         if (MASKED && !((actbits >> (R0 + i)) & 1u)) e[R0 + i] = 0.0;
         if (ETRICK)
             Dp = fma(cu[i], e[R0 + i], Dp);
@@ -103,13 +109,15 @@
 template <int R, int B, int R0, int MODE, bool MASKED>
 __device__ __forceinline__ void exp_rows(double (&cA)[B], double (&uA)[B], double (&cB)[B], double (&uB)[B],
                                          const TabRef tr, double (&e)[R], double& Dp,
-                                         const double* cbase, const double* ubase, uint32_t actbits) {
+                                         const double* cbase, const double* ubase, uint32_t actbits,
+                                         double* e0w, uint32_t wbits) {
     if constexpr (R0 + B < R) {
         exp_batch<R, B, R0, true, MODE, MASKED>(cA, uA, tr, e, Dp, cbase + R0 + B,
-                                                ubase + (R0 + B) * TILE_N, cB, uB, actbits);
-        exp_rows<R, B, R0 + B, MODE, MASKED>(cB, uB, cA, uA, tr, e, Dp, cbase, ubase, actbits);
+                                                ubase + (R0 + B) * TILE_N, cB, uB, actbits, e0w, wbits);
+        exp_rows<R, B, R0 + B, MODE, MASKED>(cB, uB, cA, uA, tr, e, Dp, cbase, ubase, actbits, e0w, wbits);
     } else {
-        exp_batch<R, B, R0, false, MODE, MASKED>(cA, uA, tr, e, Dp, nullptr, nullptr, cB, uB, actbits);
+        exp_batch<R, B, R0, false, MODE, MASKED>(cA, uA, tr, e, Dp, nullptr, nullptr, cB, uB, actbits, e0w,
+                                                 wbits);
     }
 }
 
@@ -138,9 +146,11 @@
     asm volatile("barrier.cluster.arrive.release.aligned;\n\tbarrier.cluster.wait.acquire.aligned;" ::: "memory");
 }
 
-template <int R, bool FULL, int CW, int BATCH, int MODE, int CL, bool WST = false, int M = 1>
+template <int R, bool FULL, int CW, int BATCH, int MODE, int CL, bool WST = false, int M = 1, bool E0 = false>
 __global__ void __launch_bounds__(CW * 32, 1) pass_fused_kernel(const FusedParams p) {
     static_assert(M == 1 || ((MODE & 2) && R <= 16 && !WST), "M = 2 needs the multiplicative constant and R <= 16");
+    static_assert(!E0 || (MODE == 3 && M == 1 && !WST), "the exp(-u') cache serves plain multiplicative passes");
+    constexpr bool E0W = MODE == 3 && M == 1 && !WST && !E0;
     extern __shared__ __align__(128) unsigned char smem_raw[];
     if (p.loop && *reinterpret_cast<volatile int*>(&p.loop->done)) return;
     const int K = p.K;
@@ -172,7 +182,7 @@
     }
     for (int i = threadIdx.x; i < 2 * M * SLOTS * 32; i += blockDim.x) xD[i] = 0.0;
     const uint32_t tabRep = (smem_u32(stages + (size_t)p.NS * p.stageBytes) + 8191u) & ~8191u;
-    if (MODE & 1)
+    if ((MODE & 1) && !E0)
         for (int i = threadIdx.x; i < 32 * 32; i += blockDim.x)
             asm volatile("st.shared.f64 [%0], %1;" ::"r"(tabRep + i * 8), "d"(MBAR_EXP_TABLE[i >> 5]));
     if (threadIdx.x == 0) {
@@ -197,6 +207,7 @@
     const int g = warp / p.Wk, w = warp % p.Wk;
     const int k0 = w * p.Rw;
 
+    const unsigned char* const src0 = reinterpret_cast<const unsigned char*>(E0 ? p.e0 : p.u);
     auto issue = [&](int it2, int slot2, int wrap2) {
         const int64_t s2 = (int64_t)grp + (int64_t)it2 * nGroups;
         if (s2 >= p.nStages) return;
@@ -210,17 +221,14 @@
         } else if (CL == 1) {
             const uint32_t bytes = (uint32_t)ntl * p.tileBytes;
             mbar_arrive_expect_tx(fb, bytes);
-            const unsigned char* src =
-                reinterpret_cast<const unsigned char*>(p.u) + (size_t)tile0 * p.tileBytes;
+            const unsigned char* src = src0 + (size_t)tile0 * p.tileBytes;
             for (uint32_t off = 0; off < bytes; off += FUSED_COPY_CHUNK)
                 bulk_g2s(dst + off, src + off, min(FUSED_COPY_CHUNK, bytes - off), fb);
         } else {
             const uint32_t tb = (uint32_t)Kl * TILE_N * 8;
             mbar_arrive_expect_tx(fb, (uint32_t)ntl * tb);
             for (int64_t t = 0; t < ntl; ++t)
-                bulk_g2s(dst + (uint32_t)t * tb,
-                         reinterpret_cast<const unsigned char*>(p.u) + (size_t)(tile0 + t) * p.tileBytes +
-                             (size_t)kbase * TILE_N * 8,
+                bulk_g2s(dst + (uint32_t)t * tb, src0 + (size_t)(tile0 + t) * p.tileBytes + (size_t)kbase * TILE_N * 8,
                          tb, fb);
         }
     };
@@ -233,6 +241,11 @@
             const int k = kbase + k0 + r;
             if (r < p.Rw && k0 + r < Kl && ((p.rowmask[k >> 6] >> (k & 63)) & 1ull)) actbits |= 1u << r;
         }
+        double* const e0base = (E0W && p.e0mode == E0_WRITE) ? p.e0 + (size_t)(kbase + k0) * TILE_N + lane : nullptr;
+        uint32_t wbits = 0;
+#pragma unroll
+        for (int r = 0; r < R; ++r)
+            if (r < p.Rw && k0 + r < Kl) wbits |= 1u << r;
         int par = 0;
         int it = 0;
         double mprod = 1.0;
@@ -259,7 +272,14 @@
                 const double wn = (!FULL && p.wgt) ? __ldg(p.wgt + tile * TILE_N + lane) : 1.0;
                 double e[R];
                 double Dp = 0.0;
-                {
+                if constexpr (E0) {
+#pragma unroll
+                    for (int r = 0; r < R; ++r) {
+                        e[r] = tp[r * TILE_N];
+                        if (!FULL && !((actbits >> r) & 1u)) e[r] = 0.0;
+                        Dp = fma(c_s[k0 + r], e[r], Dp);
+                    }
+                } else {
                     constexpr int B = R < BATCH ? R : BATCH;
                     double cA[B], uA[B], cB[B], uB[B];
 #pragma unroll
@@ -267,7 +287,8 @@
                         uA[i] = lds_f64(tp + i * TILE_N);
                         cA[i] = lds_f64(c_s + k0 + i);
                     }
-                    exp_rows<R, B, 0, MODE, !FULL>(cA, uA, cB, uB, tr, e, Dp, c_s + k0, tp, actbits);
+                    double* const e0w = E0W && e0base ? e0base + (size_t)tile * K * TILE_N : nullptr;
+                    exp_rows<R, B, 0, MODE, !FULL>(cA, uA, cB, uB, tr, e, Dp, c_s + k0, tp, actbits, e0w, wbits);
                 }
                 double D = Dp, D2 = 0.0, Dp2 = 0.0;
                 if constexpr (M == 2) {
@@ -769,6 +790,11 @@
         else if (!(p.mode & 2)) { kern = pass_fused_kernel<R_, true, 8, 8, 1, CL_, true>; which = ID_ + 2; } \
         else { kern = pass_fused_kernel<R_, true, 8, 8, 3, CL_, true>; which = ID_ + 3; }                    \
     }
+#define PICKE(R_, CL_, ID_)                                                                          \
+    if (Rt == R_ && p.CL == CL_ && p.e0mode == E0_READ) {                                            \
+        if (!full) { kern = pass_fused_kernel<R_, false, 8, 8, 3, CL_, false, 1, true>; which = ID_; } \
+        else { kern = pass_fused_kernel<R_, true, 8, 8, 3, CL_, false, 1, true>; which = ID_ + 1; }    \
+    }
 #define PICKM(R_, CL_, ID_)                                                                          \
     if (Rt == R_ && p.CL == CL_) {                                                                   \
         if (!full) { kern = pass_fused_kernel<R_, false, 8, 8, 3, CL_, false, 2>; which = ID_; }     \
@@ -782,21 +808,30 @@
         PICK(24, 1, 60) PICK(24, 2, 64) PICK(24, 4, 68) PICK(24, 8, 72)
         PICKW(32, 1, 24) PICKW(32, 2, 28) PICKW(32, 4, 32) PICKW(32, 8, 36) PICKW(16, 1, 52) PICKW(8, 1, 56)
         PICKW(24, 1, 76) PICKW(24, 2, 80) PICKW(24, 4, 84) PICKW(24, 8, 88)
+        PICKE(8, 1, 92) PICKE(16, 1, 94) PICKE(32, 1, 96) PICKE(32, 2, 98) PICKE(32, 4, 100) PICKE(32, 8, 102)
+        PICKE(24, 1, 104) PICKE(24, 2, 106) PICKE(24, 4, 108) PICKE(24, 8, 110)
     }
 #undef PICKM
+#undef PICKE
 #undef PICKW
 #undef PICK
     MBAR_REQUIRE(kern, MBAR_B200_ERR_INVALID, "no fused kernel variant for K=%d", p.K);
-    const bool isW = (which >= 24 && which < 40) || (which >= 52 && which < 60) || which >= 76;
+    const bool isW = (which >= 24 && which < 40) || (which >= 52 && which < 60) || (which >= 76 && which < 92);
     MBAR_REQUIRE(!p.Wout || isW, MBAR_B200_ERR_INVALID, "no weight-storing fused variant for K=%d", p.K);
+    MBAR_REQUIRE(p.e0mode != E0_READ || (which >= 92 && ctx->e0State == E0_VALID && p.e0 == ctx->d_e0),
+                 MBAR_B200_ERR_INVALID, "fused pass: stale exp(-u') cache");
+    MBAR_REQUIRE(p.e0mode != E0_WRITE || (!ctx->capturing && !p.debugSkip && p.e0 == ctx->d_e0 && p.M == 1 &&
+                                          (p.mode & 2) && !p.Wout),
+                 MBAR_B200_ERR_INVALID, "fused pass: bad exp(-u') cache write");
     snprintf(ctx->lastKernel, sizeof(ctx->lastKernel),
-             "pass_fused_kernel<R=%d, %s, CW=8, BATCH=8, MODE=%d (%s), CL=%d%s> grid=%lld NS=%d TPW=%d", Rt,
+             "pass_fused_kernel<R=%d, %s, CW=8, BATCH=8, MODE=%d (%s), CL=%d%s%s> grid=%lld NS=%d TPW=%d", Rt,
              full ? "FULL" : "MASKED", (p.mode & 2) ? 3 : 1,
              (p.mode & 2) ? "LDS table + multiplicative state constant" : "LDS table", p.CL,
              (which >= 40 && which < 52) ? ", M=2 (two candidates per launch)"
                            : isW ? ", WST (weights stored for the Hessian)" : "",
+             p.e0mode == E0_READ ? ", E0=read (cached exp(-u'))" : p.e0mode == E0_WRITE ? ", E0=write" : "",
              (long long)grid, p.NS, p.TPW);
-    static size_t attrSetAll[16][96] = {{0}};
+    static size_t attrSetAll[16][112] = {{0}};
     size_t* attrSet = attrSetAll[ctx->device & 15];
     if (attrSet[which] < smem) {
         MBAR_CUDA(cudaFuncSetAttribute(kern, cudaFuncAttributeMaxDynamicSharedMemorySize, (int)smem));
@@ -824,7 +859,63 @@
     ctx->launches++;
     ctx->passes++;
     MBAR_CUDA(cudaGetLastError());
+    if (p.e0mode == E0_WRITE) ctx->e0State = E0_VALID;
     return MBAR_B200_OK;
+}
+
+constexpr size_t E0_MARGIN = size_t(2) << 30;
+
+static bool e0_reserve(mbar_b200_ctx* ctx) {
+    if (ctx->d_e0) return true;
+    const size_t bytes = (size_t)ctx->nTiles * ctx->K * TILE_N * sizeof(double);
+    size_t freeB = 0, totalB = 0;
+    if (cudaMemGetInfo(&freeB, &totalB) != cudaSuccess) {
+        cudaGetLastError();
+        return false;
+    }
+    const size_t wt = (ctx->d_Wt || ctx->wtAllocFailed) ? 0 : bytes;
+    if (freeB < bytes + wt + E0_MARGIN) return false;
+    if (cudaMalloc((void**)&ctx->d_e0, bytes) != cudaSuccess) {
+        cudaGetLastError();
+        ctx->d_e0 = nullptr;
+        return false;
+    }
+    return true;
+}
+
+void e0_select(mbar_b200_ctx* ctx, FusedParams& p, bool mayWrite) {
+    p.e0 = nullptr;
+    p.e0mode = E0_OFF;
+    if (p.M != 1 || !(p.mode & 2) || p.Wout) return;
+    if (ctx->e0State == E0_VALID) {
+        p.e0 = ctx->d_e0;
+        p.e0mode = E0_READ;
+        return;
+    }
+    if (!mayWrite || p.debugSkip || ctx->capturing || ctx->e0State == E0_NO_ROOM) return;
+    if (ctx->e0Passes++ < 1) return;
+    if (!e0_reserve(ctx)) {
+        ctx->e0State = E0_NO_ROOM;
+        return;
+    }
+    p.e0 = ctx->d_e0;
+    p.e0mode = E0_WRITE;
+}
+
+void e0_invalidate(mbar_b200_ctx* ctx) {
+    ctx->e0State = E0_NONE;
+    ctx->e0Passes = 0;
+}
+
+void e0_release(mbar_b200_ctx* ctx) {
+    if (ctx->d_e0) {
+        cudaSetDevice(ctx->device);
+        if (ctx->stream) cudaStreamSynchronize(ctx->stream);
+        cudaFree(ctx->d_e0);
+        cudaGetLastError();
+    }
+    ctx->d_e0 = nullptr;
+    if (ctx->e0State == E0_VALID) ctx->e0State = E0_NONE;
 }
 
 int launch_pass_fused(mbar_b200_ctx* ctx, const double* h_f, bool wantL, bool allStates, bool* usedOut,
@@ -834,6 +925,7 @@
     MBAR_TRY(fused_prepare(ctx, h_f, wantL, allStates, &p, usedOut, nullptr, nullptr, wantW));
     if (!*usedOut) return MBAR_B200_OK;
     if (wroteW) *wroteW = p.Wout != nullptr;
+    e0_select(ctx, p, true);
     return fused_enqueue(ctx, p);
 }
 
```

After: 392.1 billion (median of 6 runs). No clear change (+0.2%).
